# thegenemyers/FASTGA

Hardware: NVIDIA H100
Metric: Gbp aligned/sec (genome x genome) (higher is better)
Workload: dtype int32

## Files before the change

### fastga_b200/csrc/api.cu

```cuda
#include "stages.h"
#include "handles.h"
#include <vector>
#include <algorithm>
#include <string.h>
#include <chrono>

typedef unsigned long long u64;

static inline long long now_us()
{ return std::chrono::duration_cast<std::chrono::microseconds>(std::chrono::steady_clock::now().time_since_epoch()).count(); }

static fgb_timings g_timings;

struct stage_timer
{ cudaEvent_t a, b; cudaStream_t st; float *dst;
  stage_timer(float *d, cudaStream_t s) : st(s), dst(d)
    { cudaEventCreate(&a); cudaEventCreate(&b); cudaEventRecord(a,st); }
  ~stage_timer()
    { cudaEventRecord(b,st); cudaEventSynchronize(b);
      float ms = 0; cudaEventElapsedTime(&ms,a,b); *dst += ms;
      cudaEventDestroy(a); cudaEventDestroy(b);
    }
};

void fgb_timing_add(int which, float ms)
{ if (which == 0) g_timings.triples_ms += ms;
  else if (which == 1) { g_timings.extend_ms += ms; g_timings.extend_launches += 1; }
  else if (which == 3) { g_timings.merge_ms += ms; g_timings.merge_launches += 1; }
  else g_timings.d2h_ms += ms;
}

void fgb_count_launch(int n) { g_timings.launches += n; }


#include <map>
#include <unordered_map>
#include <mutex>

static std::multimap<size_t,void *> g_free;
static std::unordered_map<void *,size_t> g_live;
static std::mutex g_mem_lock;

static size_t size_class(size_t b)
{ if (b < 4096) return 4096;
  size_t p = 4096;
  while (p < b) p <<= 1;
  size_t step = p >> 4;
  return ((b + step - 1) / step) * step;
}

cudaError_t fgb_dmalloc(void **p, size_t bytes, cudaStream_t st)
{ (void) st;
  size_t c = size_class(bytes);
  std::lock_guard<std::mutex> g(g_mem_lock);
  auto it = g_free.lower_bound(c);
  if (it != g_free.end() && it->first <= c + (c >> 2))
    { *p = it->second;
      g_live[*p] = it->first;
      g_free.erase(it);
      return cudaSuccess;
    }
  cudaError_t e = cudaMalloc(p,c);
  if (e != cudaSuccess)
    { cudaGetLastError();
      for (auto &kv : g_free) cudaFree(kv.second);
      g_free.clear();
      e = cudaMalloc(p,c);
      if (e != cudaSuccess) return e;
    }
  g_live[*p] = c;
  return cudaSuccess;
}

void fgb_dfree(void *p, cudaStream_t st)
{ (void) st;
  if (p == NULL) return;
  std::lock_guard<std::mutex> g(g_mem_lock);
  auto it = g_live.find(p);
  if (it == g_live.end()) { cudaFree(p); return; }
  g_free.insert(std::make_pair(it->second,p));
  g_live.erase(it);
}

extern "C" void fgb_release_cache()
{ std::lock_guard<std::mutex> g(g_mem_lock);
  for (auto &kv : g_free) cudaFree(kv.second);
  g_free.clear();
}

extern "C" int fgb_device_alloc(long long bytes, void **out, void *stream)
{ CUDA_TRY(fgb_dmalloc(out,(size_t) (bytes > 0 ? bytes : 16),(cudaStream_t) stream)); return FGB_OK; }
extern "C" void fgb_device_free(void *p) { fgb_dfree(p,0); }

extern "C" long long fgb_device_live_bytes()
{ std::lock_guard<std::mutex> g(g_mem_lock);
  long long s = 0;
  for (auto &kv : g_live) s += (long long) kv.second;
  return s;
}

extern "C" void fgb_timings_reset() { memset(&g_timings,0,sizeof(g_timings)); }
extern "C" void fgb_timings_get(fgb_timings *out) { *out = g_timings; }


static const long long *g_sort_len;
static int LSORT(const void *l, const void *r)
{ int x = *((const int *) l), y = *((const int *) r);
  return (int) (g_sort_len[y] - g_sort_len[x]);
}

extern "C" int fgb_genome_create(const unsigned char *bps, long long bps_bytes, int ncontig,
                                 const long long *clen, const long long *boff, int want_revcomp,
                                 fgb_genome **out, void *stream)
{ cudaStream_t st = (cudaStream_t) stream;
  if (ncontig <= 0 || ncontig > 0x7fff) return FGB_ERR_LIMIT;
  std::unique_ptr<fgb_genome> g(new fgb_genome());
  g->ncontig = ncontig;
  g->clen.assign(clen,clen+ncontig);
  g->boff.assign(boff,boff+ncontig);
  g->woff.resize(ncontig+1);
  g->seqtot = 0; g->maxlen = 0;
  long long w = 2;
  for (int c = 0; c < ncontig; c++)
    { if (clen[c] >= 0x7fffffffll) return FGB_ERR_LIMIT;
      g->woff[c] = w;
      w += ((clen[c] + 31) >> 5) + 2;
      w = (w + 1) & ~1ll;
      g->seqtot += clen[c];
      if (clen[c] > g->maxlen) g->maxlen = clen[c];
    }
  g->woff[ncontig] = w;
  g->total_words = w;

  g->perm.resize(ncontig); g->crank.resize(ncontig);
  for (int c = 0; c < ncontig; c++) g->perm[c] = c;
  g_sort_len = clen;
  qsort(g->perm.data(),ncontig,sizeof(int),LSORT);
  for (int c = 0; c < ncontig; c++) g->crank[g->perm[c]] = c;

  dblock<unsigned char> d_bps;
  dblock<long long> d_boff;
  CUDA_TRY(d_bps.alloc(bps_bytes + 16,st));
  CUDA_TRY(d_boff.alloc(ncontig,st));
  CUDA_TRY(g->d_clen.alloc(ncontig,st));
  CUDA_TRY(g->d_woff.alloc(ncontig+1,st));
  CUDA_TRY(g->d_crank.alloc(ncontig,st));
  CUDA_TRY(g->d_perm.alloc(ncontig,st));
  CUDA_TRY(g->d_seq.alloc(w + 1024,st));
  if (want_revcomp) CUDA_TRY(g->d_rseq.alloc(w + 1024,st));
  { stage_timer t(&g_timings.h2d_ms,st);
    CUDA_TRY(cudaMemcpyAsync(d_bps,bps,bps_bytes,cudaMemcpyHostToDevice,st));
    CUDA_TRY(cudaMemcpyAsync(d_boff,boff,sizeof(long long)*ncontig,cudaMemcpyHostToDevice,st));
    CUDA_TRY(cudaMemcpyAsync(g->d_clen,clen,sizeof(long long)*ncontig,cudaMemcpyHostToDevice,st));
    CUDA_TRY(cudaMemcpyAsync(g->d_woff,g->woff.data(),sizeof(long long)*(ncontig+1),cudaMemcpyHostToDevice,st));
    CUDA_TRY(cudaMemcpyAsync(g->d_crank,g->crank.data(),sizeof(int)*ncontig,cudaMemcpyHostToDevice,st));
    CUDA_TRY(cudaMemcpyAsync(g->d_perm,g->perm.data(),sizeof(int)*ncontig,cudaMemcpyHostToDevice,st));
  }
  g->h2d_bytes = bps_bytes + (long long) ncontig*(3*8+2*4) + 8;
  int rc;
  { stage_timer t(&g_timings.stage_ms,st);
    rc = fgb_stage_genome_device(d_bps,d_boff,g->d_clen,g->d_woff,ncontig,w,g->d_seq,g->d_rseq,st);
  }
  CUDA_TRY(cudaStreamSynchronize(st));
  if (rc) return rc;
  *out = g.release();
  return FGB_OK;
}

extern "C" void fgb_genome_free(fgb_genome *g) { delete g; }

extern "C" int fgb_genome_perm(const fgb_genome *g, int *perm_out)
{ memcpy(perm_out,g->perm.data(),sizeof(int)*g->ncontig); return FGB_OK; }

extern "C" int fgb_genome_download(const fgb_genome *g, int rev, unsigned long long *words,
                                   long long *woff_out)
{ const u64 *src = rev ? g->d_rseq : g->d_seq;
  if (src == NULL) return FGB_ERR_ARG;
  CUDA_TRY(cudaMemcpy(words,src,sizeof(u64)*g->total_words,cudaMemcpyDeviceToHost));
  memcpy(woff_out,g->woff.data(),sizeof(long long)*(g->ncontig+1));
  return FGB_OK;
}
extern "C" long long fgb_genome_words(const fgb_genome *g) { return g->total_words; }


extern "C" void fgb_gix_free(fgb_gix *x) { delete x; }

static void gix_bytes(const fgb_genome *g, fgb_gix *x)
{ long long cum;
  x->post_bytes = 0;
  for (cum = 1; cum < g->maxlen; cum *= 256) x->post_bytes += 1;
  x->cont_bytes = 0;
  for (cum = 1; cum < 2ll*g->ncontig; cum *= 256) x->cont_bytes += 1;
}


#define GIX_FWD_ONLY 0x80000000u

struct scan_layout
{ int fsh = 0, dbits = 0;
  dblock<unsigned long long> hist;
};

static int gix_scan(const fgb_genome *g, const unsigned char *mask, unsigned plo, unsigned phi_flags,
                    dblock<rec128> &d_recs, long long *n_out, long long *nrev, unsigned long long *buck1024,
                    scan_layout &lay, cudaStream_t st)
{ int T = fgb_sc_tile();
  std::vector<int> tc, ts;
  long long npos = 0;
  for (int c = 0; c < g->ncontig; c++)
    if (g->clen[c] >= 12 && g->boff[c] >= 0 && (mask == NULL || mask[c]))
      { npos += g->clen[c] - 11;
        for (long long t0 = 0; t0 + 12 <= g->clen[c]; t0 += T)
          { tc.push_back(c); ts.push_back((int) t0); }
      }
  int ntiles = (int) tc.size();
  dblock<int> d_tc, d_ts; dblock<unsigned> d_cnt;
  dblock<u64> d_buck, d_total; dblock<unsigned char> d_tmp;
  int rc;
  u64 total = 0, rdropped = 0;
  const unsigned phi = phi_flags & ~GIX_FWD_ONLY;
  fgb_kmer_first_digit(2*npos,plo,phi > plo ? phi : plo + 1,&lay.fsh,&lay.dbits);
  const long long ncnt = (long long) ntiles << lay.dbits;
  const long long tmpb = fgb_dev_scan_tmp_bytes(ncnt);
  CUDA_TRY(lay.hist.alloc(256,st));
  CUDA_TRY(d_tc.alloc(ntiles+1,st));
  CUDA_TRY(d_ts.alloc(ntiles+1,st));
  CUDA_TRY(d_cnt.alloc(ncnt+1,st));
  CUDA_TRY(d_buck.alloc(1025,st));
  CUDA_TRY(d_total.alloc(1,st));
  CUDA_TRY(d_tmp.alloc(tmpb,st));
  CUDA_TRY(cudaMemcpyAsync(d_tc,tc.data(),sizeof(int)*ntiles,cudaMemcpyHostToDevice,st));
  CUDA_TRY(cudaMemcpyAsync(d_ts,ts.data(),sizeof(int)*ntiles,cudaMemcpyHostToDevice,st));
  { stage_timer t(&g_timings.scan_ms,st);
    rc = fgb_syncmer_digit_count_device(g->d_seq,g->d_clen,g->d_woff,g->d_crank,d_tc,d_ts,ntiles,d_buck,d_cnt,
                                        lay.fsh,lay.dbits,lay.hist,d_total,d_tmp,tmpb,plo,phi_flags,st);
    if (rc) return rc;
    CUDA_TRY(cudaMemcpyAsync(&total,d_total,8,cudaMemcpyDeviceToHost,st));
    if (buck1024) CUDA_TRY(cudaMemcpyAsync(buck1024,d_buck,8*1024,cudaMemcpyDeviceToHost,st));
    CUDA_TRY(cudaMemcpyAsync(&rdropped,d_buck + 1024,8,cudaMemcpyDeviceToHost,st));
    CUDA_TRY(cudaStreamSynchronize(st));
  }
  if (total >= 0xfffffff0ull) return FGB_ERR_LIMIT;
  dblock<rec128> d_a;
  CUDA_TRY(d_a.alloc(total+1,st));
  { stage_timer t(&g_timings.scan_ms,st);
    rc = fgb_syncmer_digit_emit_device(g->d_seq,g->d_clen,g->d_woff,g->d_crank,d_tc,d_ts,ntiles,d_cnt,lay.fsh,
                                       lay.dbits,(long long) total,d_a,plo,phi_flags,st);
  }
  if (rc) return rc;
  CUDA_TRY(cudaStreamSynchronize(st));
  d_recs = std::move(d_a); *n_out = (long long) total; *nrev = (long long) rdropped;
  return FGB_OK;
}

static int gix_finish(fgb_gix *x, dblock<rec128> d_a, long long n, unsigned plo, unsigned phi, const scan_layout &lay,
                      cudaStream_t st, bool index = true)
{ dblock<rec128> d_b; dblock<unsigned char> d_stmp;
  long long stmpb = fgb_sort128_tmp_bytes(n);
  int rc, inb = 0;
  x->n = n;
  CUDA_TRY(d_b.alloc(n+1,st));
  CUDA_TRY(d_stmp.alloc(stmpb,st));
  if (index)
    { CUDA_TRY(x->d_pstart.alloc((1<<24)+1+8,st));
      CUDA_TRY(x->d_adj.alloc((size_t) n + 32,st));
    }
  { stage_timer t(&g_timings.ksort_ms,st);
    rc = fgb_kmer_sort_device(d_a,d_b,n,plo,phi,lay.fsh,lay.dbits,lay.hist,d_stmp,stmpb,&inb,st);
  }
  if (rc) return rc;
  x->d_tab = std::move(inb ? d_b : d_a);
  if (index)
    { stage_timer t(&g_timings.index_ms,st);
      rc = fgb_kix_index_device(x->d_tab,n,x->d_pstart,x->d_adj,st);
    }
  if (rc) return rc;
  CUDA_TRY(cudaStreamSynchronize(st));
  return FGB_OK;
}

static int gix_build_range(const fgb_genome *g, unsigned plo, unsigned phi_flags, bool index, fgb_gix **out,
                           void *stream)
{ cudaStream_t st = (cudaStream_t) stream;
  const unsigned phi = phi_flags & ~GIX_FWD_ONLY;
  std::unique_ptr<fgb_gix> x(new fgb_gix());
  gix_bytes(g,x.get());
  x->ncontig = g->ncontig;
  x->fwd_only = (phi_flags & GIX_FWD_ONLY) ? 1 : 0;
  dblock<rec128> d_a; long long n = 0, nrev = 0;
  scan_layout lay;
  int rc = gix_scan(g,NULL,plo,phi_flags,d_a,&n,&nrev,x->buck1024,lay,st);
  if (rc) return rc;
  x->n_both = n + nrev;
  const char *part_env = getenv("FGB_KSORT_PARTITION");
  const bool ignore_layout = part_env != NULL && atoi(part_env) != 0;
  const scan_layout none;
  if ((rc = gix_finish(x.get(),std::move(d_a),n,plo,phi,ignore_layout ? none : lay,st,index))) return rc;
  *out = x.release();
  return FGB_OK;
}

extern "C" int fgb_gix_build(const fgb_genome *g, fgb_gix **out, void *stream)
{ return gix_build_range(g,0u,1u << 24,true,out,stream); }

extern "C" int fgb_gix_build_forward(const fgb_genome *g, fgb_gix **out, void *stream)
{ return gix_build_range(g,0u,(1u << 24) | GIX_FWD_ONLY,true,out,stream); }

extern "C" int fgb_gix_build_range(const fgb_genome *g, unsigned plo, unsigned phi, fgb_gix **out, void *stream)
{ if (plo > phi || phi > (1u << 24)) return FGB_ERR_ARG;
  return gix_build_range(g,plo,phi,true,out,stream);
}


extern "C" int fgb_kmers_scan(const fgb_genome *g, const unsigned char *mask, int fwd_only,
                              void **d_recs, long long *n, void *stream)
{ dblock<rec128> d; long long nrev = 0;
  scan_layout lay;
  int rc = gix_scan(g,mask,0u,(1u << 24) | (fwd_only ? GIX_FWD_ONLY : 0u),d,n,&nrev,NULL,lay,(cudaStream_t) stream);
  if (rc) return rc;
  *d_recs = d.release();
  return FGB_OK;
}

extern "C" int fgb_gix_from_records(const void *d_recs, long long n, unsigned plo, unsigned phi, int fwd_only,
                                    int post_bytes, int cont_bytes, int ncontig, fgb_gix **out, void *stream)
{ cudaStream_t st = (cudaStream_t) stream;
  if (n < 0 || n >= 0xfffffff0ll || plo >= phi || phi > (1u << 24)) return FGB_ERR_ARG;
  std::unique_ptr<fgb_gix> x(new fgb_gix());
  x->n_both = n; x->post_bytes = post_bytes; x->cont_bytes = cont_bytes; x->ncontig = ncontig;
  x->fwd_only = fwd_only ? 1 : 0;
  dblock<rec128> d_a;
  CUDA_TRY(d_a.alloc(n+1,st));
  if (n > 0) CUDA_TRY(cudaMemcpyAsync(d_a,d_recs,sizeof(rec128)*n,cudaMemcpyDeviceToDevice,st));
  int rc = gix_finish(x.get(),std::move(d_a),n,plo,phi,scan_layout(),st);
  if (rc) return rc;
  *out = x.release();
  return FGB_OK;
}

extern "C" long long fgb_gix_size(const fgb_gix *x) { return x->n; }
extern "C" int fgb_gix_post_bytes(const fgb_gix *x) { return x->post_bytes; }
extern "C" int fgb_gix_cont_bytes(const fgb_gix *x) { return x->cont_bytes; }

extern "C" int fgb_gix_download(const fgb_gix *x, void *tab , unsigned *pstart ,
                                unsigned long long *buck1024)
{ if (tab) CUDA_TRY(cudaMemcpy(tab,x->d_tab,sizeof(rec128)*x->n,cudaMemcpyDeviceToHost));
  if (pstart) CUDA_TRY(cudaMemcpy(pstart,x->d_pstart,sizeof(unsigned)*((1<<24)+1),cudaMemcpyDeviceToHost));
  if (buck1024) memcpy(buck1024,x->buck1024,8*1024);
  return FGB_OK;
}

extern "C" int fgb_gix_upload(const void *tab, long long n, int post_bytes, int cont_bytes,
                              int ncontig, fgb_gix **out, void *stream)
{ cudaStream_t st = (cudaStream_t) stream;
  if (n >= 0xfffffff0ll) return FGB_ERR_LIMIT;
  std::unique_ptr<fgb_gix> x(new fgb_gix());
  x->n = n; x->n_both = n; x->post_bytes = post_bytes; x->cont_bytes = cont_bytes; x->ncontig = ncontig;
  CUDA_TRY(x->d_tab.alloc(n+1,st));
  CUDA_TRY(x->d_pstart.alloc((1<<24)+1+8,st));
  CUDA_TRY(x->d_adj.alloc((size_t) x->n + 32,st));
  CUDA_TRY(cudaMemcpyAsync(x->d_tab,tab,sizeof(rec128)*n,cudaMemcpyHostToDevice,st));
  int rc = fgb_kix_index_device(x->d_tab,n,x->d_pstart,x->d_adj,st);
  CUDA_TRY(cudaStreamSynchronize(st));
  if (rc) return rc;
  *out = x.release();
  return FGB_OK;
}

extern "C" int fgb_gix_import_ktab(const unsigned char *entries, long long n, int post_bytes,
                                   int cont_bytes, const long long *index, int ncontig,
                                   fgb_gix **out, void *stream)
{ cudaStream_t st = (cudaStream_t) stream;
  if (n >= 0xfffffff0ll || post_bytes > 4 || cont_bytes > 2) return FGB_ERR_LIMIT;
  std::unique_ptr<fgb_gix> x(new fgb_gix());
  x->n = n; x->n_both = n; x->post_bytes = post_bytes; x->cont_bytes = cont_bytes; x->ncontig = ncontig;
  long long E = 9 + post_bytes + cont_bytes;
  dblock<unsigned char> d_ent; dblock<long long> d_index;
  CUDA_TRY(d_ent.alloc(E*n + 16,st));
  CUDA_TRY(d_index.alloc(1ll << 24,st));
  CUDA_TRY(x->d_tab.alloc(n+1,st));
  CUDA_TRY(x->d_pstart.alloc((1<<24)+1+8,st));
  CUDA_TRY(x->d_adj.alloc((size_t) x->n + 32,st));
  CUDA_TRY(cudaMemcpyAsync(d_ent,entries,E*n,cudaMemcpyHostToDevice,st));
  CUDA_TRY(cudaMemcpyAsync(d_index,index,8ll<<24,cudaMemcpyHostToDevice,st));
  int rc = fgb_ktab_import_device(d_ent,n,post_bytes,cont_bytes,d_index,x->d_tab,st);
  if (!rc) rc = fgb_kix_index_device(x->d_tab,n,x->d_pstart,x->d_adj,st);
  CUDA_TRY(cudaStreamSynchronize(st));
  if (rc) return rc;
  *out = x.release();
  return FGB_OK;
}

extern "C" int fgb_gix_export_ktab(const fgb_gix *x, const long long *part_first, int nparts,
                                   unsigned char *out, void *stream)
{ cudaStream_t st = (cudaStream_t) stream;
  long long E = 9 + x->post_bytes + x->cont_bytes;
  dblock<unsigned char> d_out; dblock<long long> d_pf;
  CUDA_TRY(d_out.alloc(E*x->n + 16,st));
  CUDA_TRY(d_pf.alloc(nparts+1,st));
  CUDA_TRY(cudaMemcpyAsync(d_pf,part_first,8*nparts,cudaMemcpyHostToDevice,st));
  int rc = fgb_ktab_export_device(x->d_tab,x->n,x->post_bytes,x->cont_bytes,d_pf,nparts,d_out,st);
  if (!rc) CUDA_TRY(cudaMemcpyAsync(out,d_out,E*x->n,cudaMemcpyDeviceToHost,st));
  CUDA_TRY(cudaStreamSynchronize(st));
  return rc;
}


static int bitlen(long long v) { int b = 0; while (v > 0) { b += 1; v >>= 1; } return b; }

extern "C" void fgb_seeds_free(fgb_seeds *s) { delete s; }

static int seeds_find_impl(const fgb_gix *x1, const fgb_gix *x2, long long amxpos,
                           long long bmxpos, int freq, bool self, fgb_seeds **out, void *stream);

extern "C" int fgb_seeds_find(const fgb_gix *x1, const fgb_gix *x2, long long amxpos,
                              long long bmxpos, int freq, fgb_seeds **out, void *stream)
{ return seeds_find_impl(x1,x2,amxpos,bmxpos,freq,false,out,stream); }

extern "C" int fgb_seeds_find_self(const fgb_gix *x, long long amxpos, int freq, fgb_seeds **out, void *stream)
{ return seeds_find_impl(x,x,amxpos,amxpos,freq,true,out,stream); }

struct seed_bits { int anti, band, jc, ic, key; };

static int seed_layout_of(const fgb_gix *x1, const fgb_gix *x2, long long amxpos, long long bmxpos, seed_bits *L)
{ L->anti = bitlen(amxpos + bmxpos);
  L->band = L->anti > 6 ? L->anti - 6 : 1;
  L->jc   = bitlen(x2->ncontig > 1 ? x2->ncontig-1 : 1);
  L->ic   = bitlen(x1->ncontig > 1 ? x1->ncontig-1 : 1);
  L->key  = 12 + L->anti + L->band + L->jc + L->ic + 1;
  return L->key > 128 ? FGB_ERR_LIMIT : FGB_OK;
}

static int seeds_merge_impl(const fgb_gix *x1, const fgb_gix *x2, long long amxpos, long long bmxpos, int freq,
                            bool self, const seed_bits &L, dblock<rec128> &d_out, long long *nseeds_out,
                            long long *sumlen_out, long long *n1m_out, cudaStream_t st)
{ if (self && x1->fwd_only) return FGB_ERR_ARG;
  dblock<u64> d_counters; dblock<rec128> d_fwd, d_a;
  int rc;
  u64 nseeds = 0, sumlen = 0;
  const rec128 *t1 = x1->d_tab; long long n1 = x1->n;
  CUDA_TRY(d_counters.alloc(2,st));
  if (!self && !x1->fwd_only && n1 > 0)
    { CUDA_TRY(d_fwd.alloc(n1+1,st));
      if ((rc = fgb_forward_view_device(x1->d_tab,n1,d_fwd,&n1,st))) return rc;
      t1 = d_fwd;
    }
  long long cap = (self ? 2*x1->n : 2*n1 + (n1 >> 1)) + 1024;
  for (int attempt = 0; ; attempt++)
    { CUDA_TRY(d_a.alloc(cap+1,st));
      if (self)
        rc = fgb_self_merge_device(x1->d_tab,x1->n,x1->d_pstart,freq,L.anti,L.band,L.jc,L.ic,amxpos,
                                   d_a,cap,d_counters,&nseeds,&sumlen,st);
      else
        rc = fgb_merge_device(t1,n1,x2->d_tab,x2->n,x2->d_pstart,x2->d_adj,freq,L.anti,L.band,L.jc,L.ic,
                              amxpos,bmxpos,d_a,cap,d_counters,&nseeds,&sumlen,st);
      if (rc == FGB_OK) break;
      d_a.reset();
      if (rc != FGB_ERR_OVERFLOW || attempt > 0) return rc;
      cap = (long long) nseeds + 1024;
      g_timings.merge_ms = 0; g_timings.merge_launches = 0;
    }
  if (nseeds >= 0xfffffff0ull) return FGB_ERR_LIMIT;
  d_out = std::move(d_a); *nseeds_out = (long long) nseeds; *sumlen_out = (long long) sumlen; *n1m_out = n1;
  return FGB_OK;
}

#define SEED_SORT_LO_ANY    6
#define SEED_SORT_LO_MERGED 7

static int seeds_sort_impl(dblock<rec128> d_a, long long n, const seed_bits &L, int bit_lo, long long amxpos,
                           long long bmxpos, bool self, long long sumlen, long long n1m, fgb_seeds **out,
                           cudaStream_t st)
{ dblock<rec128> d_b; dblock<unsigned char> d_tmp;
  std::unique_ptr<fgb_seeds> s(new fgb_seeds());
  s->self_mode = self ? 1 : 0;
  s->anti_bits = L.anti; s->band_bits = L.band; s->jc_bits = L.jc; s->ic_bits = L.ic;
  s->amxpos = amxpos; s->bmxpos = bmxpos;
  s->n = n; s->sumlen = sumlen; s->n1_merged = n1m;
  long long tmpb = fgb_sort128_tmp_bytes(n);
  int rc, inb = 0;
  const char *wide_env = getenv("FGB_SEED_SORT_WIDE");
  const bool narrow = L.key <= 64 && !(wide_env != NULL && atoi(wide_env) != 0);
  u64 hiflag = 0, *d_hiflag = NULL;
  CUDA_TRY(d_b.alloc(n+1,st));
  CUDA_TRY(d_tmp.alloc(tmpb,st));
  { stage_timer t(&g_timings.ssort_ms,st);
    rc = fgb_radix_sort_device(d_a,d_b,n,bit_lo,L.key,narrow,d_tmp,tmpb,&inb,&d_hiflag,st);
  }
  if (rc) return rc;
  if (d_hiflag) CUDA_TRY(cudaMemcpyAsync(&hiflag,d_hiflag,8,cudaMemcpyDeviceToHost,st));
  CUDA_TRY(cudaStreamSynchronize(st));
  if (hiflag) return FGB_ERR_ARG;
  s->d_rec = std::move(inb ? d_b : d_a);
  *out = s.release();
  return FGB_OK;
}

static int seeds_find_impl(const fgb_gix *x1, const fgb_gix *x2, long long amxpos,
                           long long bmxpos, int freq, bool self, fgb_seeds **out, void *stream)
{ cudaStream_t st = (cudaStream_t) stream;
  seed_bits L;
  int rc = seed_layout_of(x1,x2,amxpos,bmxpos,&L);
  if (rc) return rc;
  dblock<rec128> d_a; long long n = 0, sumlen = 0, n1m = 0;
  if ((rc = seeds_merge_impl(x1,x2,amxpos,bmxpos,freq,self,L,d_a,&n,&sumlen,&n1m,st))) return rc;
  return seeds_sort_impl(std::move(d_a),n,L,SEED_SORT_LO_MERGED,amxpos,bmxpos,self,sumlen,n1m,out,st);
}


extern "C" int fgb_seeds_merge(const fgb_gix *x1, const fgb_gix *x2, long long amxpos, long long bmxpos, int freq,
                               void **d_seeds, long long *n, int *bits, long long *info, void *stream)
{ seed_bits L;
  int rc = seed_layout_of(x1,x2,amxpos,bmxpos,&L);
  if (rc) return rc;
  dblock<rec128> d_a; long long sumlen = 0, n1m = 0;
  if ((rc = seeds_merge_impl(x1,x2,amxpos,bmxpos,freq,false,L,d_a,n,&sumlen,&n1m,(cudaStream_t) stream))) return rc;
  *d_seeds = d_a.release();
  bits[0] = L.anti; bits[1] = L.band; bits[2] = L.jc; bits[3] = L.ic;
  if (info) { info[0] = sumlen; info[1] = n1m; }
  return FGB_OK;
}

static int group_by_owner(const void *d_src, long long n, int pos, int nbits, const int *owner, int nowner,
                          int world, void *d_out, long long *bounds, cudaStream_t st)
{ if (world < 1 || world > 64) return FGB_ERR_ARG;
  for (int w = 0; w <= world; w++) bounds[w] = 0;
  if (n <= 0) return FGB_OK;
  dblock<int> d_owner; dblock<u64> d_cnt;
  int rc;
  u64 cnt[64], base[65];
  CUDA_TRY(d_owner.alloc((size_t) nowner,st));
  CUDA_TRY(d_cnt.alloc(64*2,st));
  CUDA_TRY(cudaMemcpyAsync(d_owner,owner,sizeof(int)*(size_t) nowner,cudaMemcpyHostToDevice,st));
  CUDA_TRY(cudaMemsetAsync(d_cnt,0,8*64*2,st));
  if ((rc = fgb_owner_count_device(d_src,n,pos,nbits,d_owner,nowner,world,d_cnt,st))) return rc;
  CUDA_TRY(cudaMemcpyAsync(cnt,d_cnt,8*64,cudaMemcpyDeviceToHost,st));
  CUDA_TRY(cudaStreamSynchronize(st));
  base[0] = 0;
  for (int w = 0; w < world; w++) base[w+1] = base[w] + cnt[w];
  CUDA_TRY(cudaMemcpyAsync(d_cnt + 64,base,8*64,cudaMemcpyHostToDevice,st));
  if ((rc = fgb_owner_scatter_device(d_src,n,pos,nbits,d_owner,nowner,world,d_cnt + 64,d_out,st))) return rc;
  CUDA_TRY(cudaStreamSynchronize(st));
  for (int w = 0; w <= world; w++) bounds[w] = (long long) base[w];
  return FGB_OK;
}

extern "C" int fgb_seeds_group_by_owner(const void *d_seeds, long long n, const int *bits, const int *owner,
                                        int nrank_contigs, int world, void *d_out, long long *bounds,
                                        void *stream)
{ return group_by_owner(d_seeds,n,12 + bits[0] + bits[1] + bits[2],bits[3],owner,nrank_contigs,world,d_out,bounds,
                        (cudaStream_t) stream);
}

extern "C" int fgb_records_group_by_owner(const void *d_recs, long long n, const int *owner256, int world,
                                          void *d_out, long long *bounds, void *stream)
{ return group_by_owner(d_recs,n,120,8,owner256,256,world,d_out,bounds,(cudaStream_t) stream); }

extern "C" int fgb_seeds_from_records(const void *d_recs, long long n, const int *bits, long long amxpos,
                                      long long bmxpos, long long sumlen, fgb_seeds **out, void *stream)
{ cudaStream_t st = (cudaStream_t) stream;
  if (n < 0 || n >= 0xfffffff0ll) return FGB_ERR_LIMIT;
  seed_bits L;
  L.anti = bits[0]; L.band = bits[1]; L.jc = bits[2]; L.ic = bits[3];
  L.key = 12 + L.anti + L.band + L.jc + L.ic + 1;
  if (L.key > 128) return FGB_ERR_LIMIT;
  dblock<rec128> d_a;
  CUDA_TRY(d_a.alloc(n+1,st));
  if (n > 0) CUDA_TRY(cudaMemcpyAsync(d_a,d_recs,sizeof(rec128)*n,cudaMemcpyDeviceToDevice,st));
  return seeds_sort_impl(std::move(d_a),n,L,SEED_SORT_LO_ANY,amxpos,bmxpos,false,sumlen,0,out,st);
}

extern "C" long long fgb_seeds_size(const fgb_seeds *s) { return s->n; }
extern "C" long long fgb_seeds_sumlen(const fgb_seeds *s) { return s->sumlen; }
extern "C" int fgb_seeds_layout(const fgb_seeds *s, int *bits )
{ bits[0] = s->anti_bits; bits[1] = s->band_bits; bits[2] = s->jc_bits; bits[3] = s->ic_bits; return FGB_OK; }
extern "C" int fgb_seeds_download(const fgb_seeds *s, void *rec)
{ CUDA_TRY(cudaMemcpy(rec,s->d_rec,sizeof(rec128)*s->n,cudaMemcpyDeviceToHost)); return FGB_OK; }

extern "C" int fgb_sort128_host(void *recs, long long n, int byte_lo, int byte_hi, void *stream)
{ cudaStream_t st = (cudaStream_t) stream;
  dblock<rec128> d_a, d_b; dblock<unsigned char> d_tmp;
  long long tmpb = fgb_sort128_tmp_bytes(n);
  CUDA_TRY(d_a.alloc(n+1,st));
  CUDA_TRY(d_b.alloc(n+1,st));
  CUDA_TRY(d_tmp.alloc(tmpb,st));
  CUDA_TRY(cudaMemcpyAsync(d_a,recs,sizeof(rec128)*n,cudaMemcpyHostToDevice,st));
  int inb = 0;
  int rc = fgb_sort128_device(d_a,d_b,n,byte_lo,byte_hi,d_tmp,tmpb,&inb,st);
  if (!rc) CUDA_TRY(cudaMemcpyAsync(recs,inb ? d_b : d_a,sizeof(rec128)*n,cudaMemcpyDeviceToHost,st));
  CUDA_TRY(cudaStreamSynchronize(st));
  return rc;
}

extern "C" int fgb_device_ready()
{ int n = 0;
  if (cudaGetDeviceCount(&n) != cudaSuccess || n == 0) return 0;
  return 1;
}


struct fgb_run_stats
{ long long nkmers1, nkmers2, nseeds, sumlen, nhits, nla, nwaves, ncells, nraw, h2d_bytes, d2h_bytes,
            nseg, nwork, warp_cycles, wave_cycles, extract_cycles,
            us_gix, us_seeds, us_extend, us_filter, nkmers1_fwd,
            slow_cycles, slow_waves, paired_waves, pairings; };

static int align_pipeline(const fgb_genome *A, const fgb_genome *B, bool self, const float *freqA, int freq,
                          int chain_break, int chain_min, int align_min, double align_rate, fgb_alns **out,
                          fgb_run_stats *stats, cudaStream_t st)
{ fgb_run_stats s = {};
  fgb_seeds *ps = NULL; fgb_overlaps *po = NULL;
  int rc;
  long long t0 = now_us(), t1, t2, t3, t4;
  { std::unique_ptr<fgb_gix> x1, x2;
    fgb_gix *p = NULL;
    if ((rc = gix_build_range(A,0u,(1u << 24) | (self ? 0u : GIX_FWD_ONLY),self,&p,st))) return rc;
    x1.reset(p);
    if (!self)
      { if ((rc = gix_build_range(B,0u,1u << 24,true,&p,st))) return rc;
        x2.reset(p);
      }
    const fgb_gix *xb = self ? x1.get() : x2.get();
    t1 = now_us();
    s.nkmers1 = x1->n_both; s.nkmers2 = xb->n;
    seed_bits L;
    dblock<rec128> d_a; long long n = 0;
    rc = seed_layout_of(x1.get(),xb,A->maxlen,B->maxlen,&L);
    if (!rc) rc = seeds_merge_impl(x1.get(),xb,A->maxlen,B->maxlen,freq,self,L,d_a,&n,&s.sumlen,&s.nkmers1_fwd,st);
    x1.reset(); x2.reset();
    if (!rc) rc = seeds_sort_impl(std::move(d_a),n,L,SEED_SORT_LO_MERGED,A->maxlen,B->maxlen,self,s.sumlen,
                                  s.nkmers1_fwd,&ps,st);
  }
  if (rc) return rc;
  std::unique_ptr<fgb_seeds> sd(ps);
  s.nseeds = sd->n;
  t2 = now_us();
  std::vector<short> tables(65536);
  int ave = 0;
  fgb_align_spec(1.-align_rate,freqA,tables.data(),&ave);
  rc = fgb_extend(sd.get(),A,B,chain_break,chain_min,align_min,align_rate,tables.data(),ave,100,&po,st);
  t3 = now_us();
  const int jb = sd->jc_bits, ib = sd->ic_bits;
  sd.reset();
  if (rc) return rc;
  std::unique_ptr<fgb_overlaps> ov(po);
  rc = fgb_filter(ov.get(),A->perm.data(),B->perm.data(),jb,ib,1,out);
  t4 = now_us();
  unsigned long long c[16];
  fgb_overlaps_counters(ov.get(),c);
  s.us_gix = t1-t0; s.us_seeds = t2-t1; s.us_extend = t3-t2; s.us_filter = t4-t3;
  s.nhits = (long long) c[0]; s.nla = (long long) c[1]; s.nwaves = (long long) c[2]; s.ncells = (long long) c[3];
  s.nseg = (long long) c[5]; s.nwork = (long long) c[6];
  s.warp_cycles = (long long) c[8]; s.wave_cycles = (long long) c[9]; s.extract_cycles = (long long) c[10];
  s.slow_cycles = (long long) ((c[15] >> 40) << 12); s.slow_waves = (long long) ((c[15] >> 16) & 0xffffff);
  s.paired_waves = (long long) c[11]; s.pairings = (long long) c[12];
  s.h2d_bytes = A->h2d_bytes + (self ? 0 : B->h2d_bytes) + 65536*2;
  s.d2h_bytes = fgb_overlaps_bytes(ov.get()) + 16 + 8*1024*(self ? 1 : 2) + 64;
  if (stats) *stats = s;
  return rc;
}

extern "C" int fgb_align_resident(const fgb_genome *A, const fgb_genome *B, const float *freqA,
                                  int freq, int chain_break, int chain_min, int align_min,
                                  double align_rate, fgb_alns **out, fgb_run_stats *stats, void *stream)
{ return align_pipeline(A,B,false,freqA,freq,chain_break,chain_min,align_min,align_rate,out,stats,
                        (cudaStream_t) stream);
}

extern "C" int fgb_fastga_self(const unsigned char *bps, long long nb, int nc, const long long *clen,
                               const long long *boff, const float *freq4,
                               int freq, int chain_break, int chain_min, int align_min, double align_rate,
                               fgb_alns **out, fgb_run_stats *stats, void *stream)
{ fgb_genome *p = NULL;
  int rc;
  if ((rc = fgb_genome_create(bps,nb,nc,clen,boff,1,&p,stream))) return rc;
  std::unique_ptr<fgb_genome> A(p);
  return align_pipeline(A.get(),A.get(),true,freq4,freq,chain_break,chain_min,align_min,align_rate,out,stats,
                        (cudaStream_t) stream);
}

extern "C" int fgb_fastga(const unsigned char *bpsA, long long nbA, int ncA, const long long *clenA,
                          const long long *boffA, const float *freqA,
                          const unsigned char *bpsB, long long nbB, int ncB, const long long *clenB,
                          const long long *boffB,
                          int freq, int chain_break, int chain_min, int align_min, double align_rate,
                          fgb_alns **out, fgb_run_stats *stats, void *stream)
{ fgb_genome *p = NULL;
  int rc;
  if ((rc = fgb_genome_create(bpsA,nbA,ncA,clenA,boffA,1,&p,stream))) return rc;
  std::unique_ptr<fgb_genome> A(p);
  if ((rc = fgb_genome_create(bpsB,nbB,ncB,clenB,boffB,0,&p,stream))) return rc;
  std::unique_ptr<fgb_genome> B(p);
  return align_pipeline(A.get(),B.get(),false,freqA,freq,chain_break,chain_min,align_min,align_rate,out,stats,
                        (cudaStream_t) stream);
}
```

### fastga_b200/csrc/common.cuh

```cuda
#pragma once
#include <cuda_runtime.h>
#include <stdint.h>
#include <stdio.h>
#include <stdlib.h>

#define FGB_OK            0
#define FGB_ERR_CUDA     -1
#define FGB_ERR_ARG      -2
#define FGB_ERR_LIMIT    -3
#define FGB_ERR_OVERFLOW -4

#define CUDA_TRY(call)                                                                   \
  do { cudaError_t _e = (call);                                                          \
       if (_e != cudaSuccess)                                                            \
         { fprintf(stderr,"fastga_b200: CUDA error %s at %s:%d: %s\n",                   \
                   cudaGetErrorName(_e),__FILE__,__LINE__,cudaGetErrorString(_e));       \
           return FGB_ERR_CUDA; } } while (0)

struct __align__(16) rec128 { unsigned long long lo, hi; };

static __device__ __forceinline__ rec128 ld_rec(const rec128 *p)
{ uint4 v = *reinterpret_cast<const uint4 *>(p);
  rec128 r;
  r.lo = (unsigned long long) v.x | ((unsigned long long) v.y << 32);
  r.hi = (unsigned long long) v.z | ((unsigned long long) v.w << 32);
  return r;
}

static __device__ __forceinline__ void st_rec(rec128 *p, rec128 r)
{ uint4 v;
  v.x = (unsigned) r.lo; v.y = (unsigned) (r.lo >> 32);
  v.z = (unsigned) r.hi; v.w = (unsigned) (r.hi >> 32);
  *reinterpret_cast<uint4 *>(p) = v;
}

static __device__ __forceinline__ unsigned rec_byte(const rec128 &r, int b)
{ return (b < 8) ? (unsigned) ((r.lo >> (8*b)) & 0xff) : (unsigned) ((r.hi >> (8*(b-8))) & 0xff); }

static __device__ __forceinline__ unsigned rec_dig(const rec128 &r, int sh)
{ if (sh >= 64) return (unsigned) ((r.hi >> (sh - 64)) & 0xff);
  if (sh <= 56) return (unsigned) ((r.lo >> sh) & 0xff);
  return (unsigned) (((r.lo >> sh) | (r.hi << (64 - sh))) & 0xff);
}

static __device__ __forceinline__ unsigned lanemask_lt()
{ unsigned m; asm volatile("mov.u32 %0, %%lanemask_lt;" : "=r"(m)); return m; }

#define KREC_PREFIX24(hi)   ((unsigned) ((hi) >> 40))
#define KREC_SUFFIX56(r)    ((((r).hi & 0xffffffffffull) << 16) | ((r).lo >> 48))

int fgb_dev_exclusive_scan_u32(unsigned *d_data, long long n, unsigned long long *d_total,
                               void *d_tmp, long long tmp_bytes, cudaStream_t st);
long long fgb_dev_scan_tmp_bytes(long long n);

void fgb_timing_add(int which, float ms);
void fgb_count_launch(int n);

cudaError_t fgb_dmalloc(void **p, size_t bytes, cudaStream_t st);
void fgb_dfree(void *p, cudaStream_t st);

template<class T> struct dblock
{ dblock() = default;
  dblock(const dblock &) = delete;
  dblock &operator=(const dblock &) = delete;
  dblock(dblock &&o) noexcept : p(o.p), st(o.st) { o.p = nullptr; }
  dblock &operator=(dblock &&o) noexcept
    { if (this != &o) { reset(); p = o.p; st = o.st; o.p = nullptr; } return *this; }
  ~dblock() { reset(); }
  cudaError_t alloc(size_t count, cudaStream_t s)
    { reset();
      void *q = nullptr;
      cudaError_t e = fgb_dmalloc(&q,sizeof(T)*count,s);
      if (e == cudaSuccess) { p = (T *) q; st = s; }
      return e;
    }
  void reset() { if (p != nullptr) { fgb_dfree(p,st); p = nullptr; } }
  T *release() { T *q = p; p = nullptr; return q; }
  operator T *() const { return p; }
private:
  T *p = nullptr;
  cudaStream_t st = 0;
};

static __device__ __forceinline__ unsigned smem_u32(const void *p)
{ return (unsigned) __cvta_generic_to_shared(p); }

static __device__ __forceinline__ void mbar_init(unsigned long long *bar, int count)
{ asm volatile("mbarrier.init.shared::cta.b64 [%0], %1;" :: "r"(smem_u32(bar)), "r"(count) : "memory");
  asm volatile("fence.mbarrier_init.release.cluster;" ::: "memory");
  asm volatile("fence.proxy.async.shared::cta;" ::: "memory");
}

static __device__ __forceinline__ void tma_load_1d(void *smem_dst, const void *gmem_src, unsigned bytes,
                                                   unsigned long long *bar)
{ asm volatile("mbarrier.arrive.expect_tx.shared::cta.b64 _, [%0], %1;"
               :: "r"(smem_u32(bar)), "r"(bytes) : "memory");
  asm volatile("cp.async.bulk.shared::cluster.global.mbarrier::complete_tx::bytes [%0], [%1], %2, [%3];"
               :: "r"(smem_u32(smem_dst)), "l"(gmem_src), "r"(bytes), "r"(smem_u32(bar)) : "memory");
}

static __device__ __forceinline__ void mbar_expect_tx(unsigned long long *bar, unsigned bytes)
{ asm volatile("mbarrier.arrive.expect_tx.shared::cta.b64 _, [%0], %1;"
               :: "r"(smem_u32(bar)), "r"(bytes) : "memory");
}

static __device__ __forceinline__ void tma_copy_1d(void *smem_dst, const void *gmem_src, unsigned bytes,
                                                   unsigned long long *bar)
{ asm volatile("cp.async.bulk.shared::cluster.global.mbarrier::complete_tx::bytes [%0], [%1], %2, [%3];"
               :: "r"(smem_u32(smem_dst)), "l"(gmem_src), "r"(bytes), "r"(smem_u32(bar)) : "memory");
}

static __device__ __forceinline__ void mbar_wait(unsigned long long *bar, unsigned phase)
{ unsigned ok;
  do
    asm volatile("{ .reg .pred p; mbarrier.try_wait.parity.shared::cta.b64 p, [%1], %2; selp.u32 %0, 1, 0, p; }"
                 : "=r"(ok) : "r"(smem_u32(bar)), "r"(phase) : "memory");
  while (!ok);
}
```

### fastga_b200/csrc/sort128.cu

```cuda
#include "stages.h"
#include <stdlib.h>
#include <utility>
#include <vector>

#define SORT_THREADS 512
#ifndef SORT_ITEMS
#define SORT_ITEMS   8
#endif
#ifndef SORT64_ITEMS
#define SORT64_ITEMS 16
#endif
#ifndef SORT_MINBLK
#define SORT_MINBLK  2
#endif
#define SORT_TILE    (SORT_THREADS*SORT_ITEMS)
#define SORT_WARPS   (SORT_THREADS/32)
static_assert(SORT_THREADS*SORT64_ITEMS >= SORT_TILE, "fgb_sort128_tmp_bytes sizes the look-back status for SORT_TILE");

typedef unsigned long long u64;

static __device__ __forceinline__ unsigned warp_incl_scan(unsigned v, int lane)
{
#pragma unroll
  for (int o = 1; o < 32; o <<= 1)
    { unsigned t = __shfl_up_sync(0xffffffffu,v,o);
      if (lane >= o) v += t;
    }
  return v;
}

static __device__ __forceinline__ unsigned rec_dig(u64 v, int sh) { return (unsigned) (v >> sh) & 0xff; }
static __device__ __forceinline__ u64 ld_rec(const u64 *p) { return *p; }
static __device__ __forceinline__ void st_rec(u64 *p, u64 v) { *p = v; }



static __device__ __forceinline__ unsigned match_digit(unsigned d, bool valid)
{ unsigned peers = __ballot_sync(0xffffffffu,valid);
#pragma unroll
  for (int k = 0; k < 8; k++)
    { bool bit = (d >> k) & 1;
      unsigned bk = __ballot_sync(0xffffffffu,bit);
      peers &= bit ? bk : ~bk;
    }
  return peers;
}

static __device__ __forceinline__ unsigned warp_rank(unsigned *myc, unsigned d, bool valid)
{ const int lane = threadIdx.x & 31;
  unsigned peers = match_digit(d,valid);
  int leader = valid ? __ffs(peers)-1 : lane;
  unsigned b = 0;
  if (valid && lane == leader)
    { b = myc[d];
      myc[d] = b + __popc(peers);
    }
  b = __shfl_sync(0xffffffffu,b,leader);
  __syncwarp();
  return b + __popc(peers & lanemask_lt());
}

template <class F>
static __device__ __forceinline__ unsigned digit_offsets(unsigned *wcount, unsigned *bexcl, unsigned *wtot, F publish)
{ const int tid = threadIdx.x, lane = tid & 31, w = tid >> 5;
  unsigned c = 0, inc = 0;
  __syncthreads();
  if (tid < 256)
    {
#pragma unroll
      for (int ww = 0; ww < SORT_WARPS; ww++)
        { unsigned t = wcount[ww*256+tid];
          wcount[ww*256+tid] = c;
          c += t;
        }
      publish(c);
      inc = warp_incl_scan(c,lane);
      if (lane == 31) wtot[w] = inc;
    }
  __syncthreads();
  if (tid < 256)
    { unsigned pre = 0;
      for (int i = 0; i < w; i++) pre += wtot[i];
      bexcl[tid] = pre + inc - c;
    }
  __syncthreads();
  return c;
}

#define ST_AGG  (1ull << 62)
#define ST_INC  (2ull << 62)
#define ST_MASK ((1ull << 62) - 1)

static __device__ __forceinline__ u64 lookback(const u64 *status, unsigned tileid, int tid)
{ volatile const u64 *stt = status;
  u64 excl = 0;
  for (long long t = (long long) tileid - 1; t >= 0; )
    { u64 v[4];
#pragma unroll
      for (int q = 0; q < 4; q++)
        v[q] = (t - q >= 0) ? stt[(u64) (t - q)*256 + tid] : ST_INC;
      bool done = false;
#pragma unroll
      for (int q = 0; q < 4; q++)
        { if (done || (v[q] >> 62) == 0) break;
          excl += v[q] & ST_MASK;
          t -= 1;
          if (v[q] & ST_INC) done = true;
        }
      if (done) break;
    }
  return excl;
}

__global__ void __launch_bounds__(SORT_THREADS)
sort_ghist_kernel(const rec128 *__restrict__ in, long long n, int dsh , unsigned long long *__restrict__ ghist)
{ __shared__ unsigned h[256];
  int tid = threadIdx.x;
  if (tid < 256) h[tid] = 0;
  __syncthreads();
  const bool one = (dsh >= 64 || dsh <= 56);
  const unsigned long long *half = reinterpret_cast<const unsigned long long *>(in) + (dsh >= 64);
  const int sh = dsh & 63;
  for (long long tile0 = (long long) blockIdx.x * SORT_TILE; tile0 < n; tile0 += (long long) gridDim.x * SORT_TILE)
    {
#pragma unroll
      for (int it = 0; it < SORT_ITEMS; it++)
        { long long idx = tile0 + it*SORT_THREADS + tid;
          bool valid = idx < n;
          unsigned d = 0;
          if (valid) d = one ? (unsigned) ((half[2*idx] >> sh) & 0xff) : rec_dig(ld_rec(in + idx),dsh);
          unsigned peers = match_digit(d,valid);
          if (valid && (tid & 31) == __ffs(peers)-1) atomicAdd(&h[d],__popc(peers));
        }
    }
  __syncthreads();
  if (tid < 256 && h[tid]) atomicAdd(&ghist[tid],(unsigned long long) h[tid]);
}

__global__ void sort_bins_kernel(const unsigned long long *__restrict__ ghist, unsigned long long *__restrict__ binbase,
                                 unsigned long long *__restrict__ nexthist, unsigned *__restrict__ ticket)
{ __shared__ unsigned long long ws[8];
  int tid = threadIdx.x, lane = tid & 31, w = tid >> 5;
  unsigned long long v = ghist[tid], inc = v;
  for (int o = 1; o < 32; o <<= 1)
    { unsigned long long t = __shfl_up_sync(0xffffffffu,inc,o);
      if (lane >= o) inc += t;
    }
  if (lane == 31) ws[w] = inc;
  __syncthreads();
  unsigned long long pre = 0;
  for (int i = 0; i < w; i++) pre += ws[i];
  binbase[tid] = pre + inc - v;
  nexthist[tid] = 0;
  if (tid == 0) *ticket = 0;
}

template <int IW> struct os_tile
{ static constexpr int ITEMS = (IW == 16) ? SORT_ITEMS : SORT64_ITEMS;
  static constexpr int TILE  = SORT_THREADS*ITEMS;
  static constexpr size_t SMEM = (size_t) TILE*IW + (SORT_WARPS*256 + 256 + 256 + 8)*sizeof(unsigned)
                                 + 256*sizeof(u64);
};

template <class Key, int IW, int OW>
__global__ void __launch_bounds__(SORT_THREADS,SORT_MINBLK)
sort_onesweep_kernel(const void *__restrict__ in, void *__restrict__ out, long long n, int dsh ,
                     int next_dsh , const u64 *__restrict__ binbase,
                     u64 *__restrict__ nexthist, u64 *status , unsigned *__restrict__ ticket,
                     u64 *__restrict__ hiflag)
{ constexpr int ITEMS = os_tile<IW>::ITEMS, TILE = os_tile<IW>::TILE;
  extern __shared__ __align__(16) unsigned char smem_raw[];
  Key      *tile   = reinterpret_cast<Key *>(smem_raw);
  unsigned *wcount = reinterpret_cast<unsigned *>(smem_raw + (size_t) TILE*IW);
  unsigned *bexcl  = wcount + SORT_WARPS*256;
  unsigned *nhist  = bexcl + 256;
  unsigned *wtot   = nhist + 256;
  u64      *gbase  = reinterpret_cast<u64 *>(wtot + 8);
  __shared__ unsigned tile_s;
  __shared__ __align__(8) u64 tbar;

  int tid = threadIdx.x, lane = tid & 31, w = tid >> 5;
  if (tid == 0)
    { unsigned t = atomicAdd(ticket,1u);
      tile_s = t;
      long long t0 = (long long) t * TILE, rm = n - t0;
      unsigned nb = ((unsigned) (rm < TILE ? rm : TILE) * IW + 15u) & ~15u;
      mbar_init(&tbar,1);
      tma_load_1d(tile,reinterpret_cast<const unsigned char *>(in) + t0*IW,nb,&tbar);
    }
  for (int i = tid; i < SORT_WARPS*256; i += SORT_THREADS) wcount[i] = 0;
  if (tid < 256) nhist[tid] = 0;
  __syncthreads();
  const unsigned tileid = tile_s;
  long long tile0 = (long long) tileid * TILE;
  long long rem = n - tile0;
  int cnt = rem < TILE ? (int) rem : TILE;

  Key      r[ITEMS];
  unsigned rank[ITEMS];
  u64      hi_or = 0;
  int base = w*(32*ITEMS);
  unsigned *myc = wcount + w*256;
  mbar_wait(&tbar,0);
#pragma unroll
  for (int it = 0; it < ITEMS; it++)
    { int idx = base + it*32 + lane;
      bool valid = idx < cnt;
      unsigned d = 0;
      if (valid)
        { if constexpr (sizeof(Key) < IW)
            { rec128 v = ld_rec(reinterpret_cast<const rec128 *>(smem_raw) + idx);
              r[it] = v.lo;
              hi_or |= v.hi;
            }
          else
            r[it] = ld_rec(tile + idx);
          d = rec_dig(r[it],dsh);
        }
      rank[it] = warp_rank(myc,d,valid);
      if (next_dsh >= 0 && valid) atomicAdd(&nhist[rec_dig(r[it],next_dsh)],1u);
    }
  if (sizeof(Key) < IW && hi_or) atomicOr(hiflag,hi_or);

  u64 *mine = status + (u64) tileid*256 + tid;
  const unsigned c = digit_offsets(wcount,bexcl,wtot,[&](unsigned total)
    { if (tileid == 0)
        atomicExch(mine,ST_INC | total);
      else
        atomicExch(mine,ST_AGG | total);
    });

#pragma unroll
  for (int it = 0; it < ITEMS; it++)
    { int idx = base + it*32 + lane;
      if (idx < cnt)
        { unsigned d = rec_dig(r[it],dsh);
          st_rec(tile + (bexcl[d] + myc[d] + rank[it]),r[it]);
        }
    }
  if (tid < 256)
    { u64 excl = lookback(status,tileid,tid);
      if (tileid != 0) atomicExch(mine,ST_INC | (excl + c));
      gbase[tid] = binbase[tid] + excl - bexcl[tid];
      if (next_dsh >= 0 && nhist[tid]) atomicAdd(&nexthist[tid],(u64) nhist[tid]);
    }
  __syncthreads();

  for (int p = tid; p < cnt; p += SORT_THREADS)
    { Key v = ld_rec(tile + p);
      u64 o = gbase[rec_dig(v,dsh)] + p;
      if constexpr (sizeof(Key) < OW)
        { rec128 R; R.lo = v; R.hi = 0;
          st_rec(reinterpret_cast<rec128 *>(out) + o,R);
        }
      else
        st_rec(reinterpret_cast<Key *>(out) + o,v);
    }
}

struct sort_tmp
{ u64 *status, *hist[2], *binbase, *hiflag;
  unsigned *ticket;
  sort_tmp(void *d_tmp, long long n)
    { long long ntiles = (n + SORT_TILE - 1) / SORT_TILE;
      if (ntiles < 1) ntiles = 1;
      status  = (u64 *) d_tmp;
      hist[0] = status + 256ull*ntiles;
      hist[1] = hist[0] + 256;
      binbase = hist[1] + 256;
      ticket  = (unsigned *) (binbase + 256);
      hiflag  = binbase + 256 + 1;
    }
};

extern "C" long long fgb_sort128_tmp_bytes(long long n)
{ long long ntiles = (n + SORT_TILE - 1) / SORT_TILE;
  if (ntiles < 1) ntiles = 1;
  return 256*ntiles*8 + (3*256 + 16)*8;
}

static int first_pass_hist(const void *d_a, long long n, int dsh, const sort_tmp &T, cudaStream_t st)
{ CUDA_TRY(cudaMemsetAsync(T.hist[0],0,256*8,st));
  int ntiles = (int) ((n + SORT_TILE - 1) / SORT_TILE), nb = ntiles < 1184 ? ntiles : 1184;
  sort_ghist_kernel<<<nb,SORT_THREADS,0,st>>>((const rec128 *) d_a,n,dsh,T.hist[0]);
  fgb_count_launch(1);
  return FGB_OK;
}

template <class Key, int IW, int OW>
static int onesweep_pass(const void *in, void *out, long long n, int dsh, int next_dsh, const sort_tmp &T, int cur,
                         cudaStream_t st)
{ typedef os_tile<IW> O;
  static bool attr_set = false;
  if (!attr_set)
    { CUDA_TRY(cudaFuncSetAttribute(sort_onesweep_kernel<Key,IW,OW>,cudaFuncAttributeMaxDynamicSharedMemorySize,(int) O::SMEM));
      attr_set = true;
    }
  int ntiles = (int) ((n + O::TILE - 1) / O::TILE);
  sort_bins_kernel<<<1,256,0,st>>>(T.hist[cur],T.binbase,T.hist[cur^1],T.ticket);
  CUDA_TRY(cudaMemsetAsync(T.status,0,256ull*ntiles*8,st));
  sort_onesweep_kernel<Key,IW,OW><<<ntiles,SORT_THREADS,O::SMEM,st>>>(in,out,n,dsh,next_dsh,T.binbase,T.hist[cur^1],
                                                                     T.status,T.ticket,T.hiflag);
  fgb_count_launch(2);
  return FGB_OK;
}

extern "C" int fgb_radix_sort_device(void *d_a, void *d_b, long long n, int bit_lo, int bit_hi, int narrow,
                                     void *d_tmp, long long tmp_bytes, int *result_in_b, u64 **d_hiflag, void *stream)
{ cudaStream_t st = (cudaStream_t) stream;
  if (n < 0 || bit_lo < 0 || bit_hi > (narrow ? 64 : 128) || bit_lo > bit_hi) return FGB_ERR_ARG;
  if (n >= 0xffffffffll) return FGB_ERR_LIMIT;
  *result_in_b = 0;
  const sort_tmp T(d_tmp,n);
  if (narrow)
    { if (tmp_bytes < fgb_sort128_tmp_bytes(n)) return FGB_ERR_ARG;
      CUDA_TRY(cudaMemsetAsync(T.hiflag,0,8,st));
      *d_hiflag = T.hiflag;
    }
  if (n <= 1 || bit_lo == bit_hi) return FGB_OK;
  if (tmp_bytes < fgb_sort128_tmp_bytes(n)) return FGB_ERR_ARG;

  const int npass = (bit_hi - bit_lo + 7) / 8;
  const bool words = narrow && npass >= 2;
  void *half[2] = { d_b, (unsigned char *) d_b + ((8*n + 15) & ~15ll) };

  int rc = first_pass_hist(d_a,n,bit_lo,T,st);
  for (int p = 0; p < npass && rc == FGB_OK; p++)
    { const int b = bit_lo + 8*p, nd = (p + 1 < npass) ? b + 8 : -1, cur = p & 1;
      if (!words)
        rc = onesweep_pass<rec128,16,16>(cur ? d_b : d_a,cur ? d_a : d_b,n,b,nd,T,cur,st);
      else if (p == 0)
        rc = onesweep_pass<u64,16,8>(d_a,half[0],n,b,nd,T,cur,st);
      else if (nd >= 0)
        rc = onesweep_pass<u64,8,8>(half[cur^1],half[cur],n,b,nd,T,cur,st);
      else
        rc = onesweep_pass<u64,8,16>(half[cur^1],d_a,n,b,nd,T,cur,st);
    }
  if (rc) return rc;
  CUDA_TRY(cudaGetLastError());
  if (!words && (npass & 1))
    { if (narrow)
        CUDA_TRY(cudaMemcpyAsync(d_a,d_b,sizeof(rec128)*n,cudaMemcpyDeviceToDevice,st));
      else
        *result_in_b = 1;
    }
  return FGB_OK;
}

extern "C" int fgb_sort128_device(void *d_a, void *d_b, long long n, int byte_lo, int byte_hi,
                                  void *d_tmp, long long tmp_bytes, int *result_in_b, void *stream)
{ if (byte_lo < 0 || byte_hi > 16 || byte_lo > byte_hi) return FGB_ERR_ARG;
  return fgb_radix_sort_device(d_a,d_b,n,8*byte_lo,8*byte_hi,0,d_tmp,tmp_bytes,result_in_b,NULL,stream);
}


#define BK_THREADS SORT_THREADS
#define BK_ITEMS   8
#define BK_CAP     (BK_THREADS*BK_ITEMS)
#define BK_WARPS   SORT_WARPS
#define BK_SPAN    4
#define BK_SUBBITS 10
#define BK_NSUB    (BK_SPAN << BK_SUBBITS)
#define BK_MAXSUB  32

__global__ void kmer_bins_kernel(const rec128 *__restrict__ tab, long long n, int binshift, unsigned long long base,
                                 unsigned *__restrict__ bin_start, long long nbins)
{ long long i = (long long) blockIdx.x * blockDim.x + threadIdx.x;
  if (i > n) return;
  long long lo = (i == 0) ? -1 : (long long) ((tab[i-1].hi >> binshift) - base);
  long long hi = (i == n) ? nbins : (long long) ((tab[i].hi >> binshift) - base);
  if (hi > nbins) hi = nbins;
  for (long long p = lo+1; p <= hi; p++) bin_start[p] = (unsigned) i;
}


__global__ void __launch_bounds__(BK_THREADS,2)
kmer_bucket_sort_kernel(const rec128 *__restrict__ in, rec128 *__restrict__ out,
                        const uint4 *__restrict__ groups ,
                        int binshift)
{ extern __shared__ __align__(16) unsigned char smem_raw[];
  rec128   *tile   = reinterpret_cast<rec128 *>(smem_raw);
  unsigned *cnt    = reinterpret_cast<unsigned *>(tile + BK_CAP);
  unsigned *bexcl  = cnt + BK_NSUB + 32;
  unsigned *wtot   = bexcl + 256;
  __shared__ __align__(8) unsigned long long tbar;

  const int tid = threadIdx.x, lane = tid & 31, w = tid >> 5;
  const uint4 g = groups[blockIdx.x];
  const int count = (int) g.y;
  if (tid == 0)
    { mbar_init(&tbar,1);
      tma_load_1d(tile,in + g.x,(unsigned) count * 16u,&tbar);
    }
  for (int i = tid; i <= BK_NSUB; i += BK_THREADS) cnt[i] = 0;
  __syncthreads();
  mbar_wait(&tbar,0);

  rec128   r[BK_ITEMS];
  unsigned sub[BK_ITEMS], off[BK_ITEMS];
  const int base = w*(32*BK_ITEMS);
  const unsigned b0 = g.z;
  const int subshift = binshift - BK_SUBBITS;
#pragma unroll
  for (int it = 0; it < BK_ITEMS; it++)
    { int idx = base + it*32 + lane;
      if (idx < count)
        { r[it] = ld_rec(tile + idx);
          sub[it] = ((((unsigned) (r[it].hi >> binshift)) - b0) << BK_SUBBITS) | ((unsigned) (r[it].hi >> subshift) & ((1u << BK_SUBBITS)-1));
          off[it] = atomicAdd(&cnt[sub[it]],1u);
        }
    }
  __syncthreads();
  bool big = false;
  { unsigned v[8], sum = 0;
#pragma unroll
    for (int i = 0; i < 8; i++) { v[i] = cnt[8*tid+i]; big |= (v[i] > BK_MAXSUB); sum += v[i]; }
    unsigned inc = warp_incl_scan(sum,lane);
    if (lane == 31) wtot[w] = inc;
    __syncthreads();
    unsigned pre = inc - sum;
    for (int i = 0; i < w; i++) pre += wtot[i];
#pragma unroll
    for (int i = 0; i < 8; i++) { cnt[8*tid+i] = pre; pre += v[i]; }
    if (tid == BK_THREADS-1) cnt[BK_NSUB] = pre;
  }
  big = __syncthreads_or(big);

  if (!big)
    {
#pragma unroll
      for (int it = 0; it < BK_ITEMS; it++)
        { int idx = base + it*32 + lane;
          if (idx < count) st_rec(tile + (cnt[sub[it]] + off[it]),r[it]);
        }
      __syncthreads();
      for (int p = tid; p < count; p += BK_THREADS)
        { rec128 R = ld_rec(tile + p);
          unsigned sb = ((((unsigned) (R.hi >> binshift)) - b0) << BK_SUBBITS) | ((unsigned) (R.hi >> subshift) & ((1u << BK_SUBBITS)-1));
          int s = (int) cnt[sb], e = (int) cnt[sb+1], rank = 0;
          for (int q = s; q < e; q++)
            { rec128 Q = ld_rec(tile + q);
              bool less = (Q.hi < R.hi) || (Q.hi == R.hi && (Q.lo < R.lo || (Q.lo == R.lo && q < p)));
              rank += less;
            }
          st_rec(out + (g.x + s + rank),R);
        }
      return;
    }

  unsigned *wcount = cnt;
  unsigned *myc = wcount + w*256;
  unsigned rank[BK_ITEMS];
  __syncthreads();
#pragma unroll
  for (int i = 0; i < 8; i++) myc[i*32 + lane] = 0;
  __syncwarp();
  for (int byte = 0; byte < 16; byte++)
    {
#pragma unroll
      for (int it = 0; it < BK_ITEMS; it++)
        { int idx = base + it*32 + lane;
          bool valid = idx < count;
          rank[it] = warp_rank(myc,valid ? rec_byte(r[it],byte) : 0,valid);
        }
      digit_offsets(wcount,bexcl,wtot,[](unsigned) {});
#pragma unroll
      for (int it = 0; it < BK_ITEMS; it++)
        { int idx = base + it*32 + lane;
          if (idx < count)
            { unsigned d = rec_byte(r[it],byte);
              st_rec(tile + (bexcl[d] + myc[d] + rank[it]),r[it]);
            }
        }
      __syncthreads();
      if (byte + 1 < 16)
        {
#pragma unroll
          for (int it = 0; it < BK_ITEMS; it++)
            { int idx = base + it*32 + lane;
              if (idx < count) r[it] = ld_rec(tile + idx);
            }
#pragma unroll
          for (int i = 0; i < 8; i++) myc[i*32 + lane] = 0;
          __syncwarp();
        }
    }
  for (int p = tid; p < count; p += BK_THREADS)
    st_rec(out + (g.x + p),ld_rec(tile + p));
}

__global__ void kmer_copy_segments_kernel(const rec128 *__restrict__ src, rec128 *__restrict__ dst,
                                          const unsigned *__restrict__ sfrom, const unsigned *__restrict__ dfrom,
                                          const unsigned *__restrict__ pre, int nseg, long long total)
{ for (long long i = (long long) blockIdx.x * blockDim.x + threadIdx.x; i < total;
       i += (long long) gridDim.x * blockDim.x)
    { int lo = 0, hi = nseg;
      while (hi - lo > 1) { int md = (lo+hi) >> 1; if (pre[md] <= i) lo = md; else hi = md; }
      unsigned o = (unsigned) (i - pre[lo]);
      st_rec(dst + (dfrom[lo] + o),ld_rec(src + (sfrom[lo] + o)));
    }
}

static const size_t BUCKET_SMEM = BK_CAP*sizeof(rec128) + (BK_NSUB + 32 + 256 + BK_WARPS)*sizeof(unsigned);

extern "C" int fgb_kmer_bin_shift(long long n, unsigned plo, unsigned phi)
{ long long maxbins = 65536, target = 1536;
  if (getenv("FGB_KSORT_BIN_TARGET") != NULL) target = atoll(getenv("FGB_KSORT_BIN_TARGET"));
  if (target < 1) target = 1;
  while (maxbins < (1ll << 24) && n / maxbins > target) maxbins <<= 1;
  int sh = 0;
  while ((long long) ((((unsigned long long) (phi - 1) >> sh) - ((unsigned long long) plo >> sh))) >= maxbins) sh += 1;
  return sh;
}

extern "C" void fgb_kmer_first_digit(long long nmax, unsigned plo, unsigned phi, int *fsh, int *dbits)
{ *fsh = fgb_kmer_bin_shift(nmax,plo,phi);
  int bits = 24 - *fsh, passes = (bits - 9 + 7) / 8;
  if (passes < 1) passes = 1;
  *dbits = bits - 8*passes;
}

static int kmer_sort_binned(const rec128 *src, rec128 *dst, const unsigned *bins, long long nbins, int sh,
                            unsigned plo, cudaStream_t st)
{ const int binshift = 40 + sh;
  const unsigned base = plo >> sh;
  int rc = FGB_OK;
  static bool attr_set = false;
  if (!attr_set)
    { CUDA_TRY(cudaFuncSetAttribute(kmer_bucket_sort_kernel,cudaFuncAttributeMaxDynamicSharedMemorySize,
                                    (int) BUCKET_SMEM));
      attr_set = true;
    }

  std::vector<uint4> groups;
  std::vector<unsigned> ofrom, opre;
  unsigned ototal = 0;
  { unsigned gs = bins[0], gc = 0; long long gp = 0;
    for (long long p = 0; p < nbins; p++)
      { unsigned len = bins[p+1] - bins[p];
        if (len == 0) continue;
        if (len > BK_CAP)
          { if (gc) { groups.push_back(make_uint4(gs,gc,base + (unsigned) gp,0)); gc = 0; }
            ofrom.push_back(bins[p]); opre.push_back(ototal); ototal += len;
            continue;
          }
        if (gc != 0 && (gc + len > BK_CAP || p - gp >= BK_SPAN))
          { groups.push_back(make_uint4(gs,gc,base + (unsigned) gp,0)); gc = 0; }
        if (gc == 0) { gs = bins[p]; gp = p; }
        gc += len;
      }
    if (gc) groups.push_back(make_uint4(gs,gc,base + (unsigned) gp,0));
  }

  dblock<uint4> d_groups;
  if (!groups.empty())
    { CUDA_TRY(d_groups.alloc(groups.size(),st));
      CUDA_TRY(cudaMemcpyAsync(d_groups,groups.data(),sizeof(uint4)*groups.size(),cudaMemcpyHostToDevice,st));
      kmer_bucket_sort_kernel<<<(unsigned) groups.size(),BK_THREADS,BUCKET_SMEM,st>>>(src,dst,d_groups,binshift);
      fgb_count_launch(1);
      CUDA_TRY(cudaGetLastError());
    }
  if (ototal > 0)
    { int nseg = (int) ofrom.size();
      opre.push_back(ototal);
      std::vector<unsigned> cfrom(opre.begin(),opre.end()-1);
      dblock<rec128> d_c1, d_c2; dblock<unsigned char> d_ctmp; dblock<unsigned> d_seg;
      long long ctb = fgb_sort128_tmp_bytes(ototal);
      CUDA_TRY(d_c1.alloc((size_t) ototal+1,st));
      CUDA_TRY(d_c2.alloc((size_t) ototal+1,st));
      CUDA_TRY(d_ctmp.alloc(ctb,st));
      CUDA_TRY(d_seg.alloc(3*(size_t) nseg+1,st));
      CUDA_TRY(cudaMemcpyAsync(d_seg,ofrom.data(),sizeof(unsigned)*nseg,cudaMemcpyHostToDevice,st));
      CUDA_TRY(cudaMemcpyAsync(d_seg+nseg,cfrom.data(),sizeof(unsigned)*nseg,cudaMemcpyHostToDevice,st));
      CUDA_TRY(cudaMemcpyAsync(d_seg+2*nseg,opre.data(),sizeof(unsigned)*(nseg+1),cudaMemcpyHostToDevice,st));
      int nb = (int) ((ototal + 255) / 256); if (nb > 4736) nb = 4736;
      kmer_copy_segments_kernel<<<nb,256,0,st>>>(src,d_c1,d_seg,d_seg+nseg,d_seg+2*nseg,nseg,ototal);
      int cinb = 0;
      rc = fgb_sort128_device(d_c1,d_c2,ototal,0,16,d_ctmp,ctb,&cinb,st);
      if (rc) return rc;
      kmer_copy_segments_kernel<<<nb,256,0,st>>>(cinb ? d_c2 : d_c1,dst,d_seg+nseg,d_seg,d_seg+2*nseg,nseg,ototal);
      fgb_count_launch(2);
      CUDA_TRY(cudaGetLastError());
      CUDA_TRY(cudaStreamSynchronize(st));
    }
  CUDA_TRY(cudaStreamSynchronize(st));
  return FGB_OK;
}

extern "C" int fgb_kmer_sort_device(void *d_a, void *d_b, long long n, unsigned plo, unsigned phi, int fsh, int dbits,
                                    const u64 *d_hist, void *d_tmp, long long tmp_bytes, int *result_in_b, void *stream)
{ cudaStream_t st = (cudaStream_t) stream;
  *result_in_b = 0;
  if (n <= 1) return FGB_OK;
  if (n >= 0xffffffffll) return FGB_ERR_LIMIT;
  if (phi <= plo || phi > (1u << 24) || tmp_bytes < fgb_sort128_tmp_bytes(n)) return FGB_ERR_ARG;
  const int sh = fgb_kmer_bin_shift(n,plo,phi);
  if (dbits == 0) fsh = sh;
  if (sh < fsh) return FGB_ERR_ARG;
  const sort_tmp T(d_tmp,n);
  const int b0 = 64 + 40 + fsh + dbits, npass = (128 - b0 + 7) / 8;
  if (dbits == 0)
    { int rc = first_pass_hist(d_a,n,b0,T,st);
      if (rc) return rc;
    }
  else
    CUDA_TRY(cudaMemcpyAsync(T.hist[0],d_hist,256*8,cudaMemcpyDeviceToDevice,st));
  rec128 *src = (rec128 *) d_a, *dst = (rec128 *) d_b;
  for (int p = 0; p < npass; p++)
    { const int b = b0 + 8*p, nd = (p + 1 < npass) ? b + 8 : -1;
      int rc = onesweep_pass<rec128,16,16>(src,dst,n,b,nd,T,p & 1,st);
      if (rc) return rc;
      std::swap(src,dst);
    }
  CUDA_TRY(cudaGetLastError());

  const unsigned long long base = (unsigned long long) plo >> sh, fbase = (unsigned long long) plo >> fsh;
  const long long nf = (long long) (((unsigned long long) (phi - 1) >> fsh) - fbase) + 1;
  const long long nbins = (long long) (((unsigned long long) (phi - 1) >> sh) - base) + 1;
  std::vector<unsigned> fstart((size_t) nf + 1), bins((size_t) nbins + 1);
  { dblock<unsigned> d_fstart;
    CUDA_TRY(d_fstart.alloc((size_t) (nf+1),st));
    kmer_bins_kernel<<<(int) ((n + 1 + 255) / 256),256,0,st>>>(src,n,40 + fsh,fbase,d_fstart,nf);
    fgb_count_launch(1);
    CUDA_TRY(cudaMemcpyAsync(fstart.data(),d_fstart,sizeof(unsigned)*(size_t) (nf+1),cudaMemcpyDeviceToHost,st));
    CUDA_TRY(cudaStreamSynchronize(st));
  }
  for (long long p = 0; p <= nbins; p++)
    { long long f = (long long) ((base + p) << (sh - fsh)) - (long long) fbase;
      bins[p] = fstart[f < 0 ? 0 : (f > nf ? nf : f)];
    }
  int rc = kmer_sort_binned(src,dst,bins.data(),nbins,sh,plo,st);
  if (rc) return rc;
  *result_in_b = (dst == (rec128 *) d_b);
  return FGB_OK;
}


#define SCAN_THREADS 1024
#define SCAN_ITEMS   8
#define SCAN_TILE    (SCAN_THREADS*SCAN_ITEMS)

__global__ void __launch_bounds__(SCAN_THREADS)
scan_reduce_kernel(const unsigned *__restrict__ data, long long n, unsigned long long *__restrict__ sums)
{ __shared__ unsigned long long ws[32];
  long long t0 = (long long) blockIdx.x * SCAN_TILE;
  unsigned long long s = 0;
  for (int i = 0; i < SCAN_ITEMS; i++)
    { long long idx = t0 + i*SCAN_THREADS + threadIdx.x;
      if (idx < n) s += data[idx];
    }
  for (int o = 16; o > 0; o >>= 1) s += __shfl_down_sync(0xffffffffu,s,o);
  if ((threadIdx.x & 31) == 0) ws[threadIdx.x >> 5] = s;
  __syncthreads();
  if (threadIdx.x < 32)
    { s = ws[threadIdx.x];
      for (int o = 16; o > 0; o >>= 1) s += __shfl_down_sync(0xffffffffu,s,o);
      if (threadIdx.x == 0) sums[blockIdx.x] = s;
    }
}

__global__ void __launch_bounds__(1024)
scan_sums_kernel(unsigned long long *__restrict__ sums, int nb, unsigned long long *__restrict__ total)
{ __shared__ unsigned long long ws[32];
  __shared__ unsigned long long carry_s;
  int tid = threadIdx.x, lane = tid & 31, w = tid >> 5;
  if (tid == 0) carry_s = 0;
  __syncthreads();
  for (int base = 0; base < nb; base += 1024)
    { int i = base + tid;
      unsigned long long v = (i < nb) ? sums[i] : 0, inc = v;
      for (int o = 1; o < 32; o <<= 1)
        { unsigned long long t = __shfl_up_sync(0xffffffffu,inc,o);
          if (lane >= o) inc += t;
        }
      if (lane == 31) ws[w] = inc;
      __syncthreads();
      if (w == 0)
        { unsigned long long s = ws[lane], si = s;
          for (int o = 1; o < 32; o <<= 1)
            { unsigned long long t = __shfl_up_sync(0xffffffffu,si,o);
              if (lane >= o) si += t;
            }
          ws[lane] = si - s;
        }
      __syncthreads();
      unsigned long long ex = carry_s + ws[w] + inc - v;
      if (i < nb) sums[i] = ex;
      __syncthreads();
      if (tid == 1023) carry_s = ex + v;
      __syncthreads();
    }
  if (tid == 0 && total != NULL) *total = carry_s;
}

__global__ void __launch_bounds__(SCAN_THREADS)
scan_down_kernel(unsigned *__restrict__ data, long long n, const unsigned long long *__restrict__ sums)
{ __shared__ unsigned ws[32];
  int tid = threadIdx.x, lane = tid & 31, w = tid >> 5;
  long long t0 = (long long) blockIdx.x * SCAN_TILE + (long long) tid * SCAN_ITEMS;
  unsigned v[SCAN_ITEMS], s = 0;
#pragma unroll
  for (int i = 0; i < SCAN_ITEMS; i++)
    { v[i] = (t0 + i < n) ? data[t0+i] : 0;
      s += v[i];
    }
  unsigned inc = warp_incl_scan(s,lane);
  if (lane == 31) ws[w] = inc;
  __syncthreads();
  if (w == 0)
    { unsigned x = ws[lane];
      unsigned xi = warp_incl_scan(x,lane);
      ws[lane] = xi - x;
    }
  __syncthreads();
  unsigned ex = (unsigned) sums[blockIdx.x] + ws[w] + inc - s;
#pragma unroll
  for (int i = 0; i < SCAN_ITEMS; i++)
    { if (t0 + i < n) data[t0+i] = ex;
      ex += v[i];
    }
}

long long fgb_dev_scan_tmp_bytes(long long n)
{ long long nb = (n + SCAN_TILE - 1) / SCAN_TILE;
  if (nb < 1) nb = 1;
  return nb * 8 + 64;
}


int fgb_dev_exclusive_scan_u32(unsigned *d_data, long long n, unsigned long long *d_total,
                               void *d_tmp, long long tmp_bytes, cudaStream_t st)
{ if (n <= 0)
    { if (d_total) CUDA_TRY(cudaMemsetAsync(d_total,0,8,st));
      return FGB_OK;
    }
  if (tmp_bytes < fgb_dev_scan_tmp_bytes(n)) return FGB_ERR_ARG;
  int nb = (int) ((n + SCAN_TILE - 1) / SCAN_TILE);
  unsigned long long *sums = (unsigned long long *) d_tmp;
  scan_reduce_kernel<<<nb,SCAN_THREADS,0,st>>>(d_data,n,sums);
  scan_sums_kernel<<<1,1024,0,st>>>(sums,nb,d_total);
  scan_down_kernel<<<nb,SCAN_THREADS,0,st>>>(d_data,n,sums);
  fgb_count_launch(3);
  CUDA_TRY(cudaGetLastError());
  return FGB_OK;
}
```

### fastga_b200/csrc/stages.h

```cpp
#pragma once
#include "common.cuh"

struct fgb_genome;
struct fgb_seeds;
struct fgb_overlaps;
struct fgb_alns;

extern "C" {

long long fgb_sort128_tmp_bytes(long long n);
int fgb_radix_sort_device(void *d_a, void *d_b, long long n, int bit_lo, int bit_hi, int narrow,
                          void *d_tmp, long long tmp_bytes, int *result_in_b, unsigned long long **d_hiflag,
                          void *stream);
int fgb_sort128_device(void *d_a, void *d_b, long long n, int byte_lo, int byte_hi,
                       void *d_tmp, long long tmp_bytes, int *result_in_b, void *stream);
int fgb_kmer_bin_shift(long long n, unsigned plo, unsigned phi);
void fgb_kmer_first_digit(long long nmax, unsigned plo, unsigned phi, int *fsh, int *dbits);
int fgb_kmer_sort_device(void *d_a, void *d_b, long long n, unsigned plo, unsigned phi, int fsh, int dbits,
                         const unsigned long long *d_hist, void *d_tmp, long long tmp_bytes, int *result_in_b,
                         void *stream);

int fgb_stage_genome_device(const void *d_bps, const long long *d_boff, const long long *d_clen,
                            const long long *d_woff, int ncontig, long long total_words,
                            void *d_seq, void *d_rseq, void *stream);
int fgb_syncmer_digit_count_device(const void *d_seq, const long long *d_clen, const long long *d_woff,
                                   const int *d_crank, const int *d_tile_contig, const int *d_tile_start,
                                   int ntiles, unsigned long long *d_buck1024, unsigned *d_dmat, int dsh, int dbits,
                                   unsigned long long *d_nhist, unsigned long long *d_total, void *d_tmp,
                                   long long tmp_bytes, unsigned plo, unsigned phi, void *stream);
int fgb_syncmer_digit_emit_device(const void *d_seq, const long long *d_clen, const long long *d_woff,
                                  const int *d_crank, const int *d_tile_contig, const int *d_tile_start,
                                  int ntiles, unsigned *d_dmat, int dsh, int dbits, long long n, void *d_records,
                                  unsigned plo, unsigned phi, void *stream);
int fgb_kix_index_device(const void *d_tab, long long n, unsigned *d_pstart, unsigned char *d_adj, void *stream);
int fgb_ktab_export_device(const void *d_tab, long long n, int pbytes, int cbytes,
                           const long long *d_part_first, int nparts, void *d_out, void *stream);
int fgb_ktab_import_device(const void *d_ent, long long n, int pbytes, int cbytes,
                           const long long *d_index, void *d_tab, void *stream);
int fgb_sc_tile();

int fgb_forward_view_device(const void *d_T, long long n, void *d_out, long long *h_nfwd, void *stream);
int fgb_self_merge_device(const void *d_T, long long n, const unsigned *d_pstart, int freq,
                          int anti_bits, int band_bits, int jc_bits, int ic_bits,
                          long long amxpos, void *d_seeds, long long capacity,
                          unsigned long long *d_counters, unsigned long long *h_nseeds,
                          unsigned long long *h_sumlen, void *stream);
int fgb_merge_device(const void *d_T1, long long n1, const void *d_T2, long long n2, const unsigned *d_pstart2,
                     const unsigned char *d_adj2, int freq, int anti_bits, int band_bits, int jc_bits, int ic_bits,
                     long long amxpos, long long bmxpos, void *d_seeds, long long capacity,
                     unsigned long long *d_counters, unsigned long long *h_nseeds,
                     unsigned long long *h_sumlen, void *stream);
int fgb_owner_count_device(const void *d_seeds, long long n, int p_ic, int ic_bits, const int *d_owner, int nrc,
                           int world, unsigned long long *d_cnt, void *stream);
int fgb_owner_scatter_device(const void *d_seeds, long long n, int p_ic, int ic_bits, const int *d_owner, int nrc,
                             int world, unsigned long long *d_base, void *d_out, void *stream);

int fgb_extend(const fgb_seeds *S, const fgb_genome *A, const fgb_genome *B, int chain_break,
               int chain_min, int align_min, double align_rate, const short *tables, int ave_path,
               int tspace, fgb_overlaps **out, void *stream);
int fgb_align_spec(double ave_corr, const float *freq, short *tables, int *ave_path);
long long fgb_overlaps_bytes(const fgb_overlaps *o);
const unsigned char *fgb_overlaps_data(const fgb_overlaps *o);
void fgb_overlaps_counters(const fgb_overlaps *o, unsigned long long *out);
void fgb_overlaps_retry_info(const fgb_overlaps *o, long long out[4]);
int fgb_filter(const fgb_overlaps *O, const int *perm1, const int *perm2, int jc_bits, int ic_bits,
               int do_filter, fgb_alns **out);

}
```

### fastga_b200/lib.py

```python
import ctypes as C

import numpy as np

from . import load_library

c_void_p, c_int, c_ll = C.c_void_p, C.c_int, C.c_longlong

ERRORS = {-1: "CUDA runtime error", -2: "bad argument", -3: "input exceeds a device-layout limit",
          -4: "device arena overflow"}


class FgbError(RuntimeError):
    pass


def _check(rc, what):
    if rc != 0:
        raise FgbError("%s failed: %s (%d)" % (what, ERRORS.get(rc, "?"), rc))


class Timings(C.Structure):
    _fields_ = [(n, C.c_float) for n in
                ("h2d_ms", "stage_ms", "scan_ms", "ksort_ms", "index_ms", "merge_ms", "ssort_ms",
                 "triples_ms", "extend_ms", "d2h_ms", "filter_ms")] + \
               [("merge_launches", C.c_int), ("extend_launches", C.c_int), ("launches", C.c_int)]

    def asdict(self):
        return {n: getattr(self, n) for n, _ in self._fields_}


def _ptr(a):
    return a.ctypes.data_as(c_void_p)


def timings_reset():
    load_library().fgb_timings_reset()


def timings_get():
    t = Timings()
    load_library().fgb_timings_get(C.byref(t))
    return t.asdict()


def device_ready():
    return bool(load_library().fgb_device_ready())


def device_live_bytes():
    L = load_library()
    L.fgb_device_live_bytes.restype = c_ll
    L.fgb_device_live_bytes.argtypes = []
    return L.fgb_device_live_bytes()


class DeviceGenome:

    def __init__(self, genome, want_revcomp=False, stream=None):
        L = load_library()
        self.genome = genome
        self.h = c_void_p()
        L.fgb_genome_create.argtypes = [c_void_p, c_ll, c_int, c_void_p, c_void_p, c_int,
                                        C.POINTER(c_void_p), c_void_p]
        _check(L.fgb_genome_create(_ptr(genome.bps), genome.bps.size, genome.ncontig,
                                   _ptr(genome.clen), _ptr(genome.boff), int(want_revcomp),
                                   C.byref(self.h), stream), "fgb_genome_create")
        self.perm = np.zeros(genome.ncontig, dtype=np.int32)
        L.fgb_genome_perm.argtypes = [c_void_p, c_void_p]
        L.fgb_genome_perm(self.h, _ptr(self.perm))
        self.crank = np.empty_like(self.perm)
        self.crank[self.perm] = np.arange(genome.ncontig, dtype=np.int32)

    def download(self, rev=False):
        L = load_library()
        L.fgb_genome_words.restype = c_ll
        L.fgb_genome_words.argtypes = [c_void_p]
        n = L.fgb_genome_words(self.h)
        words = np.zeros(n, dtype=np.uint64)
        woff = np.zeros(self.genome.ncontig + 1, dtype=np.int64)
        L.fgb_genome_download.argtypes = [c_void_p, c_int, c_void_p, c_void_p]
        _check(L.fgb_genome_download(self.h, int(rev), _ptr(words), _ptr(woff)), "fgb_genome_download")
        return words, woff

    def close(self):
        if self.h:
            L = load_library()
            L.fgb_genome_free.argtypes = [c_void_p]
            L.fgb_genome_free(self.h)
            self.h = c_void_p()

    def __del__(self):
        try:
            self.close()
        except Exception:
            pass


class DeviceGix:

    def __init__(self, handle):
        self.h = handle

    @classmethod
    def build(cls, dgenome, stream=None):
        L = load_library()
        h = c_void_p()
        L.fgb_gix_build.argtypes = [c_void_p, C.POINTER(c_void_p), c_void_p]
        _check(L.fgb_gix_build(dgenome.h, C.byref(h), stream), "fgb_gix_build")
        return cls(h)

    @classmethod
    def build_forward(cls, dgenome, stream=None):
        L = load_library()
        h = c_void_p()
        L.fgb_gix_build_forward.argtypes = [c_void_p, C.POINTER(c_void_p), c_void_p]
        _check(L.fgb_gix_build_forward(dgenome.h, C.byref(h), stream), "fgb_gix_build_forward")
        return cls(h)

    @classmethod
    def build_range(cls, dgenome, plo, phi, stream=None):
        L = load_library()
        h = c_void_p()
        L.fgb_gix_build_range.argtypes = [c_void_p, C.c_uint, C.c_uint, C.POINTER(c_void_p), c_void_p]
        _check(L.fgb_gix_build_range(dgenome.h, plo, phi, C.byref(h), stream), "fgb_gix_build_range")
        return cls(h)

    @classmethod
    def upload(cls, tab, post_bytes, cont_bytes, ncontig, stream=None):
        L = load_library()
        h = c_void_p()
        tab = np.ascontiguousarray(tab, dtype=np.uint64).reshape(-1, 2)
        L.fgb_gix_upload.argtypes = [c_void_p, c_ll, c_int, c_int, c_int, C.POINTER(c_void_p), c_void_p]
        _check(L.fgb_gix_upload(_ptr(tab), tab.shape[0], post_bytes, cont_bytes, ncontig,
                                C.byref(h), stream), "fgb_gix_upload")
        return cls(h)

    @classmethod
    def import_ktab(cls, gixfile, stream=None):
        L = load_library()
        h = c_void_p()
        L.fgb_gix_import_ktab.argtypes = [c_void_p, c_ll, c_int, c_int, c_void_p, c_int,
                                          C.POINTER(c_void_p), c_void_p]
        ent = np.ascontiguousarray(gixfile.entries)
        idx = np.ascontiguousarray(gixfile.index, dtype=np.int64)
        _check(L.fgb_gix_import_ktab(_ptr(ent), gixfile.n, gixfile.post_bytes, gixfile.cont_bytes,
                                     _ptr(idx), gixfile.ncontig, C.byref(h), stream),
               "fgb_gix_import_ktab")
        return cls(h)

    @property
    def n(self):
        L = load_library()
        L.fgb_gix_size.restype = c_ll
        L.fgb_gix_size.argtypes = [c_void_p]
        return L.fgb_gix_size(self.h)

    @property
    def post_bytes(self):
        L = load_library()
        L.fgb_gix_post_bytes.argtypes = [c_void_p]
        return L.fgb_gix_post_bytes(self.h)

    @property
    def cont_bytes(self):
        L = load_library()
        L.fgb_gix_cont_bytes.argtypes = [c_void_p]
        return L.fgb_gix_cont_bytes(self.h)

    def download(self, want_index=True):
        L = load_library()
        n = self.n
        tab = np.zeros((n, 2), dtype=np.uint64)
        pstart = np.zeros((1 << 24) + 1, dtype=np.uint32) if want_index else None
        buck = np.zeros(1024, dtype=np.uint64)
        L.fgb_gix_download.argtypes = [c_void_p, c_void_p, c_void_p, c_void_p]
        _check(L.fgb_gix_download(self.h, _ptr(tab), _ptr(pstart) if want_index else None, _ptr(buck)),
               "fgb_gix_download")
        return tab, pstart, buck

    def export_ktab(self, part_first, stream=None):
        L = load_library()
        E = 9 + self.post_bytes + self.cont_bytes
        out = np.zeros(self.n * E, dtype=np.uint8)
        pf = np.ascontiguousarray(part_first, dtype=np.int64)
        L.fgb_gix_export_ktab.argtypes = [c_void_p, c_void_p, c_int, c_void_p, c_void_p]
        _check(L.fgb_gix_export_ktab(self.h, _ptr(pf), len(pf), _ptr(out), stream), "fgb_gix_export_ktab")
        return out

    def close(self):
        if self.h:
            L = load_library()
            L.fgb_gix_free.argtypes = [c_void_p]
            L.fgb_gix_free(self.h)
            self.h = c_void_p()

    def __del__(self):
        try:
            self.close()
        except Exception:
            pass


class DeviceSeeds:

    def __init__(self, handle):
        self.h = handle

    @classmethod
    def find(cls, gix1, gix2, amxpos, bmxpos, freq=10, stream=None):
        L = load_library()
        h = c_void_p()
        L.fgb_seeds_find.argtypes = [c_void_p, c_void_p, c_ll, c_ll, c_int, C.POINTER(c_void_p), c_void_p]
        _check(L.fgb_seeds_find(gix1.h, gix2.h, amxpos, bmxpos, freq, C.byref(h), stream), "fgb_seeds_find")
        return cls(h)

    @classmethod
    def find_self(cls, gix, amxpos, freq=10, stream=None):
        L = load_library()
        h = c_void_p()
        L.fgb_seeds_find_self.argtypes = [c_void_p, c_ll, c_int, C.POINTER(c_void_p), c_void_p]
        _check(L.fgb_seeds_find_self(gix.h, amxpos, freq, C.byref(h), stream), "fgb_seeds_find_self")
        return cls(h)

    @property
    def n(self):
        L = load_library()
        L.fgb_seeds_size.restype = c_ll
        L.fgb_seeds_size.argtypes = [c_void_p]
        return L.fgb_seeds_size(self.h)

    @property
    def sumlen(self):
        L = load_library()
        L.fgb_seeds_sumlen.restype = c_ll
        L.fgb_seeds_sumlen.argtypes = [c_void_p]
        return L.fgb_seeds_sumlen(self.h)

    @property
    def layout(self):
        L = load_library()
        bits = (c_int * 4)()
        L.fgb_seeds_layout.argtypes = [c_void_p, c_void_p]
        L.fgb_seeds_layout(self.h, bits)
        return tuple(bits)

    def download(self):
        L = load_library()
        rec = np.zeros((self.n, 2), dtype=np.uint64)
        L.fgb_seeds_download.argtypes = [c_void_p, c_void_p]
        _check(L.fgb_seeds_download(self.h, _ptr(rec)), "fgb_seeds_download")
        return rec

    def close(self):
        if self.h:
            L = load_library()
            L.fgb_seeds_free.argtypes = [c_void_p]
            L.fgb_seeds_free(self.h)
            self.h = c_void_p()

    def __del__(self):
        try:
            self.close()
        except Exception:
            pass


def sort128_host(recs, byte_lo, byte_hi, stream=None):
    L = load_library()
    assert recs.dtype == np.uint64 and recs.flags.c_contiguous and recs.shape[1] == 2
    L.fgb_sort128_host.argtypes = [c_void_p, c_ll, c_int, c_int, c_void_p]
    _check(L.fgb_sort128_host(_ptr(recs), recs.shape[0], byte_lo, byte_hi, stream), "fgb_sort128_host")
    return recs


OVL_DT = np.dtype([("triple", "i4"), ("seq", "i4"), ("pairkey", "i4"), ("abpos", "i4"), ("bbpos", "i4"),
                   ("aepos", "i4"), ("bepos", "i4"), ("diffs", "i4"), ("tlen", "i4"), ("toff", "i8")])


def align_spec(ave_corr, freq):
    L = load_library()
    tables = np.zeros(65536, dtype=np.int16)
    ave = c_int()
    f = np.ascontiguousarray(freq, dtype=np.float32)
    L.fgb_align_spec.argtypes = [C.c_double, c_void_p, c_void_p, C.POINTER(c_int)]
    _check(L.fgb_align_spec(float(ave_corr), _ptr(f), _ptr(tables), C.byref(ave)), "fgb_align_spec")
    return tables, ave.value


class DeviceOverlaps:

    def __init__(self, handle):
        self.h = handle

    @classmethod
    def extend(cls, seeds, dgenomeA, dgenomeB, freq, chain_break=2000, chain_min=170, align_min=100,
               align_rate=0.3, tspace=100, stream=None):
        L = load_library()
        tables, ave = align_spec(1.0 - align_rate, freq)
        h = c_void_p()
        L.fgb_extend.argtypes = [c_void_p, c_void_p, c_void_p, c_int, c_int, c_int, C.c_double, c_void_p,
                                 c_int, c_int, C.POINTER(c_void_p), c_void_p]
        _check(L.fgb_extend(seeds.h, dgenomeA.h, dgenomeB.h, chain_break, chain_min, align_min,
                            float(align_rate), _ptr(tables), ave, tspace, C.byref(h), stream), "fgb_extend")
        return cls(h)

    def counters(self):
        L = load_library()
        out = (C.c_ulonglong * 16)()
        L.fgb_overlaps_counters.argtypes = [c_void_p, c_void_p]
        L.fgb_overlaps_counters(self.h, out)
        v = list(out)
        return {"hits": v[0], "la_calls": v[1], "waves": v[2], "cells": v[3], "nseg": v[5], "nwork": v[6],
                "warp_cycles": v[8], "wave_cycles": v[9], "extract_cycles": v[10], "paired_waves": v[11], "pairings": v[12],
                "front_wait": v[4], "front_total": v[7], "back_wait": v[13],
                "max_warp_cycles": v[14],
                "slowest_warp": {"cycles": (v[15] >> 40) << 12, "waves": (v[15] >> 16) & 0xffffff, "la_calls": v[15] & 0xffff}}

    def retry_info(self):
        L = load_library()
        out = (C.c_longlong * 4)()
        L.fgb_overlaps_retry_info.argtypes = [c_void_p, c_void_p]
        L.fgb_overlaps_retry_info(self.h, out)
        return {"launches": out[0], "reasons": out[1], "regrowths": out[2], "reruns": out[3]}

    def records(self):
        L = load_library()
        L.fgb_overlaps_bytes.restype = c_ll
        L.fgb_overlaps_bytes.argtypes = [c_void_p]
        L.fgb_overlaps_data.restype = c_void_p
        L.fgb_overlaps_data.argtypes = [c_void_p]
        nb = L.fgb_overlaps_bytes(self.h)
        if nb == 0:
            return np.zeros(0, dtype=OVL_DT), np.zeros(0, dtype=np.uint8)
        buf = np.ctypeslib.as_array(C.cast(L.fgb_overlaps_data(self.h), C.POINTER(C.c_uint8)), shape=(nb,)).copy()
        recs = []
        off = 0
        while off < nb:
            h = np.frombuffer(buf[off:off + 40].tobytes(), dtype=np.int32)
            recs.append((h[0], h[1], h[2], h[3], h[4], h[5], h[6], h[7], h[8], off + 40))
            off += 40 + ((int(h[8]) + 7) & ~7)
        arr = np.array(recs, dtype=OVL_DT)
        order = np.lexsort((arr["seq"], arr["triple"]))
        return arr[order], buf

    def close(self):
        if self.h:
            L = load_library()
            L.fgb_overlaps_free.argtypes = [c_void_p]
            L.fgb_overlaps_free(self.h)
            self.h = c_void_p()

    def __del__(self):
        try:
            self.close()
        except Exception:
            pass


ALN_FIELDS = ("comp", "aread", "bread", "abpos", "bbpos", "aepos", "bepos", "diffs", "tlen")


class Alignments:

    def __init__(self, fields, toff, pool, nraw):
        self.fields = fields
        self.toff = toff
        self.pool = pool
        self.nraw = nraw

    def __len__(self):
        return self.fields.shape[0]

    def trace(self, i):
        return self.pool[int(self.toff[i]):int(self.toff[i]) + int(self.fields[i, 8])]

    def canonical_lines(self):
        return sorted(self.canonical_lines_unsorted())

    def canonical_lines_unsorted(self):
        out = []
        for i in range(len(self)):
            comp, ar, br, ab, bb, ae, be, df, tl = (int(x) for x in self.fields[i])
            t = self.trace(i)
            line = "A %d %d %d %d %d %d" % (ar, ab, ae, br, bb, be)
            if comp:
                line += " | R"
            line += " | D %d" % df
            line += " | T %d" % (tl // 2) + "".join(" %d" % v for v in t[1::2])
            line += " | X %d" % (tl // 2) + "".join(" %d" % v for v in t[0::2])
            out.append(line)
        return out


def filter_overlaps(ovl_handle, perm1, perm2, jc_bits, ic_bits, do_filter=True):
    L = load_library()
    h = c_void_p()
    p1 = np.ascontiguousarray(perm1, dtype=np.int32)
    p2 = np.ascontiguousarray(perm2, dtype=np.int32)
    L.fgb_filter.argtypes = [c_void_p, c_void_p, c_void_p, c_int, c_int, c_int, C.POINTER(c_void_p)]
    _check(L.fgb_filter(ovl_handle, _ptr(p1), _ptr(p2), jc_bits, ic_bits, int(do_filter), C.byref(h)),
           "fgb_filter")
    return _alns_out(h)


def overlaps_from_buffer(buf):
    L = load_library()
    h = c_void_p()
    buf = np.ascontiguousarray(buf, dtype=np.uint8)
    L.fgb_overlaps_from_buffer.argtypes = [c_void_p, c_ll, C.POINTER(c_void_p)]
    _check(L.fgb_overlaps_from_buffer(_ptr(buf), buf.size, C.byref(h)), "fgb_overlaps_from_buffer")
    return DeviceOverlaps(h)


class RunStats(C.Structure):
    _fields_ = [(n, c_ll) for n in ("nkmers1", "nkmers2", "nseeds", "sumlen", "nhits", "nla", "nwaves",
                                    "ncells", "nraw", "h2d_bytes", "d2h_bytes", "nseg", "nwork", "warp_cycles",
                                    "wave_cycles", "extract_cycles", "us_gix", "us_seeds", "us_extend", "us_filter",
                                    "nkmers1_fwd", "slow_cycles", "slow_waves", "paired_waves", "pairings")]

    def asdict(self):
        return {n: getattr(self, n) for n, _ in self._fields_}


DEFAULTS = dict(freq=10, chain_break=2000, chain_min=170, align_min=100, align_rate=0.3)


def _alns_out(h):
    L = load_library()
    for f in ("fgb_alns_count", "fgb_alns_raw_count", "fgb_alns_pool_bytes"):
        getattr(L, f).restype = c_ll
        getattr(L, f).argtypes = [c_void_p]
    n, nraw, pb = L.fgb_alns_count(h), L.fgb_alns_raw_count(h), L.fgb_alns_pool_bytes(h)
    fields = np.zeros((n, 9), dtype=np.int32)
    toff = np.zeros(n, dtype=np.int64)
    pool = np.zeros(max(pb, 1), dtype=np.uint8)
    L.fgb_alns_get.argtypes = [c_void_p, c_void_p, c_void_p, c_void_p]
    _check(L.fgb_alns_get(h, _ptr(fields), _ptr(toff), _ptr(pool)), "fgb_alns_get")
    L.fgb_alns_free.argtypes = [c_void_p]
    L.fgb_alns_free(h)
    return Alignments(fields, toff, pool, nraw)


def _whole_path(name, argtypes, args, stream, kw):
    p = dict(DEFAULTS)
    p.update(kw)
    L = load_library()
    h = c_void_p()
    st = RunStats()
    fn = getattr(L, name)
    fn.argtypes = argtypes + [c_int, c_int, c_int, c_int, C.c_double, C.POINTER(c_void_p), C.POINTER(RunStats),
                              c_void_p]
    _check(fn(*args, p["freq"], p["chain_break"], p["chain_min"], p["align_min"], float(p["align_rate"]),
              C.byref(h), C.byref(st), stream), name)
    return _alns_out(h), st.asdict()


def align_resident(dA, dB, freqA, stream=None, **kw):
    f = np.ascontiguousarray(freqA, dtype=np.float32)
    return _whole_path("fgb_align_resident", [c_void_p, c_void_p, c_void_p], (dA.h, dB.h, _ptr(f)), stream, kw)


def fastga_self(g, stream=None, **kw):
    f = np.ascontiguousarray(g.freq, dtype=np.float32)
    return _whole_path("fgb_fastga_self", [c_void_p, c_ll, c_int, c_void_p, c_void_p, c_void_p],
                       (_ptr(g.bps), g.bps.size, g.ncontig, _ptr(g.clen), _ptr(g.boff), _ptr(f)), stream, kw)


def fastga(gA, gB, stream=None, **kw):
    f = np.ascontiguousarray(gA.freq, dtype=np.float32)
    return _whole_path("fgb_fastga", [c_void_p, c_ll, c_int, c_void_p, c_void_p, c_void_p,
                                      c_void_p, c_ll, c_int, c_void_p, c_void_p],
                       (_ptr(gA.bps), gA.bps.size, gA.ncontig, _ptr(gA.clen), _ptr(gA.boff), _ptr(f),
                        _ptr(gB.bps), gB.bps.size, gB.ncontig, _ptr(gB.clen), _ptr(gB.boff)), stream, kw)


def compute_trace_pts(dA, dB, alns, tspace=100, stream=None, with_bad=False):
    L = load_library()
    h = c_void_p()
    fields = np.ascontiguousarray(alns.fields, dtype=np.int32)
    toff = np.ascontiguousarray(alns.toff, dtype=np.int64)
    pool = np.ascontiguousarray(alns.pool, dtype=np.uint8)
    L.fgb_compute_trace_pts.argtypes = [c_void_p, c_void_p, c_ll, c_void_p, c_void_p, c_void_p, c_int,
                                        C.POINTER(c_void_p), c_void_p]
    _check(L.fgb_compute_trace_pts(dA.h, dB.h, len(alns), _ptr(fields), _ptr(toff), _ptr(pool), tspace,
                                   C.byref(h), stream), "fgb_compute_trace_pts")
    L.fgb_scripts_total.restype = c_ll
    L.fgb_scripts_total.argtypes = [c_void_p]
    n, tot = len(alns), L.fgb_scripts_total(h)
    soff = np.zeros(n + 1, dtype=np.int64)
    script = np.zeros(max(tot, 1), dtype=np.int32)
    diffs = np.zeros(max(n, 1), dtype=np.int32)
    L.fgb_scripts_get.argtypes = [c_void_p, c_void_p, c_void_p, c_void_p]
    _check(L.fgb_scripts_get(h, _ptr(soff), _ptr(script), _ptr(diffs)), "fgb_scripts_get")
    L.fgb_scripts_bad.restype = c_ll
    L.fgb_scripts_bad.argtypes = [c_void_p]
    bad = L.fgb_scripts_bad(h)
    L.fgb_scripts_free.argtypes = [c_void_p]
    L.fgb_scripts_free(h)
    return (soff, script[:tot], diffs[:n]) + ((bad,) if with_bad else ())



def hit_groups_host(hrange, tinfo, hits, bands=1, slack=1000, gap=-1):
    L = load_library()
    hr = np.ascontiguousarray(hrange, dtype=np.uint32).reshape(-1, 2)
    ti = np.ascontiguousarray(tinfo, dtype=np.int32).reshape(-1, 2)
    hh = np.ascontiguousarray(hits, dtype=np.int64).reshape(-1, 2)
    cap = len(hh) + len(hr) + 1
    items = np.zeros((cap, 4), dtype=np.uint32)
    nxt = np.zeros((cap, 2), dtype=np.int64)
    L.fgb_hit_groups_host.restype = c_ll
    L.fgb_hit_groups_host.argtypes = [c_int, c_void_p, c_void_p, c_void_p, c_ll, c_int, c_ll, c_ll, c_void_p, c_void_p]
    n = L.fgb_hit_groups_host(len(hr), _ptr(hr), _ptr(ti), _ptr(hh), len(hh), bands, slack, gap, _ptr(items), _ptr(nxt))
    return items[:n].copy(), nxt[:n].copy()


CHAIN_TRIPLE_DT = np.dtype([("start", "i8"), ("end", "i8"), ("long", "i8"), ("key", "i8"), ("band", "i8"),
                            ("h0", "i8"), ("hn", "i8")])
CHAIN_HIT_DT = np.dtype([("alow", "i8"), ("ahgh", "i8"), ("dgmin", "i8"), ("dgmax", "i8")])
CHAIN_LISTLESS = 0x80000000


def chain_hits(seeds, chain_break=2000, chain_min=170, chunk=None, stream=None):
    L = load_library()
    L.fgb_chain_hits.argtypes = [c_void_p, c_int, c_int, c_ll, c_void_p, c_ll, c_void_p, c_ll, c_void_p, c_void_p]
    chunk = 1536 if chunk is None else int(chunk)
    info = np.zeros(6, dtype=np.int64)
    trip = np.zeros(1, dtype=CHAIN_TRIPLE_DT)
    hits = np.zeros(1, dtype=CHAIN_HIT_DT)
    for _ in range(2):
        rc = L.fgb_chain_hits(seeds.h, chain_break, chain_min, chunk, _ptr(trip), len(trip), _ptr(hits), len(hits),
                              _ptr(info), stream)
        if rc != -4:
            break
        trip = np.zeros(max(int(info[0]), 1), dtype=CHAIN_TRIPLE_DT)
        hits = np.zeros(max(int(info[2]), 1), dtype=CHAIN_HIT_DT)
    _check(rc, "fgb_chain_hits")
    names = ("work", "long", "slots", "reserved", "capacity", "chunks")
    return trip[:int(info[0])].copy(), hits[:int(info[2])].copy(), dict(zip(names, (int(v) for v in info)))


def device_free(ptr):
    L = load_library()
    L.fgb_device_free.argtypes = [c_void_p]
    L.fgb_device_free(c_void_p(ptr))


def kmers_scan(dgenome, mask, fwd_only, stream=None):
    L = load_library()
    ptr, n = c_void_p(), c_ll()
    m = np.ascontiguousarray(mask, dtype=np.uint8)
    L.fgb_kmers_scan.argtypes = [c_void_p, c_void_p, c_int, C.POINTER(c_void_p), C.POINTER(c_ll), c_void_p]
    _check(L.fgb_kmers_scan(dgenome.h, _ptr(m), int(fwd_only), C.byref(ptr), C.byref(n), stream), "fgb_kmers_scan")
    return ptr.value, n.value


def records_group_by_owner(src_ptr, n, owner256, world, dst_ptr, stream=None):
    L = load_library()
    bounds = np.zeros(world + 1, dtype=np.int64)
    own = np.ascontiguousarray(owner256, dtype=np.int32)
    assert own.shape == (256,)
    L.fgb_records_group_by_owner.argtypes = [c_void_p, c_ll, c_void_p, c_int, c_void_p, c_void_p, c_void_p]
    _check(L.fgb_records_group_by_owner(c_void_p(src_ptr), n, _ptr(own), world, c_void_p(dst_ptr), _ptr(bounds),
                                        stream), "fgb_records_group_by_owner")
    return bounds


def gix_from_records(ptr, n, plo, phi, fwd_only, post_bytes, cont_bytes, ncontig, stream=None):
    L = load_library()
    h = c_void_p()
    L.fgb_gix_from_records.argtypes = [c_void_p, c_ll, C.c_uint, C.c_uint, c_int, c_int, c_int, c_int,
                                       C.POINTER(c_void_p), c_void_p]
    _check(L.fgb_gix_from_records(c_void_p(ptr), n, plo, phi, int(fwd_only), post_bytes, cont_bytes, ncontig,
                                  C.byref(h), stream), "fgb_gix_from_records")
    return DeviceGix(h)


def seeds_merge(gix1, gix2, amxpos, bmxpos, freq=10, stream=None):
    L = load_library()
    ptr, n = c_void_p(), c_ll()
    bits = (c_int * 4)()
    info = (c_ll * 2)()
    L.fgb_seeds_merge.argtypes = [c_void_p, c_void_p, c_ll, c_ll, c_int, C.POINTER(c_void_p), C.POINTER(c_ll),
                                  c_void_p, c_void_p, c_void_p]
    _check(L.fgb_seeds_merge(gix1.h, gix2.h, amxpos, bmxpos, freq, C.byref(ptr), C.byref(n), bits, info, stream),
           "fgb_seeds_merge")
    return ptr.value, n.value, tuple(bits), info[0], info[1]


def seeds_group_by_owner(src_ptr, n, bits, owner_by_rank, world, dst_ptr, stream=None):
    L = load_library()
    bounds = np.zeros(world + 1, dtype=np.int64)
    b = (c_int * 4)(*bits)
    ow = np.ascontiguousarray(owner_by_rank, dtype=np.int32)
    L.fgb_seeds_group_by_owner.argtypes = [c_void_p, c_ll, c_void_p, c_void_p, c_int, c_int, c_void_p, c_void_p, c_void_p]
    _check(L.fgb_seeds_group_by_owner(c_void_p(src_ptr), n, b, _ptr(ow), len(ow), world, c_void_p(dst_ptr),
                                      _ptr(bounds), stream), "fgb_seeds_group_by_owner")
    return bounds


def seeds_from_records(ptr, n, bits, amxpos, bmxpos, sumlen=0, stream=None):
    L = load_library()
    h = c_void_p()
    b = (c_int * 4)(*bits)
    L.fgb_seeds_from_records.argtypes = [c_void_p, c_ll, c_void_p, c_ll, c_ll, c_ll, C.POINTER(c_void_p), c_void_p]
    _check(L.fgb_seeds_from_records(c_void_p(ptr), n, b, amxpos, bmxpos, sumlen, C.byref(h), stream),
           "fgb_seeds_from_records")
    return DeviceSeeds(h)


def local_alignments(dA, dB, jobs, freq, align_rate=0.3, tspace=100, stream=None):
    L = load_library()
    jobs = np.ascontiguousarray(jobs, dtype=np.int32).reshape(-1, 8)
    n = jobs.shape[0]
    tables, ave = align_spec(1.0 - align_rate, freq)
    paths = np.zeros((max(n, 1), 7), dtype=np.int32)
    toff = np.zeros(max(n, 1), dtype=np.int64)
    cap = 1 << 20
    L.fgb_local_alignments.argtypes = [c_void_p, c_void_p, c_ll, c_void_p, c_void_p, c_int, c_int,
                                       c_void_p, c_void_p, c_void_p, c_ll, C.POINTER(c_ll), c_void_p]
    while True:
        traces = np.zeros(cap, dtype=np.uint8)
        used = c_ll()
        rc = L.fgb_local_alignments(dA.h, dB.h, n, _ptr(jobs), _ptr(tables), ave, tspace, _ptr(paths), _ptr(toff),
                                    _ptr(traces), cap, C.byref(used), stream)
        if rc == -4 and used.value > cap:
            cap = used.value + 1024
            continue
        _check(rc, "fgb_local_alignments")
        return paths[:n], toff[:n], traces[:used.value]
```

### include/fastga_b200.h

```cpp
#ifndef FASTGA_B200_H
#define FASTGA_B200_H

#include <stdint.h>

#ifdef __cplusplus
extern "C" {
#endif

#define FGB_OK            0
#define FGB_ERR_CUDA     -1
#define FGB_ERR_ARG      -2
#define FGB_ERR_LIMIT    -3
#define FGB_ERR_OVERFLOW -4

typedef struct fgb_genome   fgb_genome;
typedef struct fgb_gix      fgb_gix;
typedef struct fgb_seeds    fgb_seeds;
typedef struct fgb_overlaps fgb_overlaps;
typedef struct fgb_alns     fgb_alns;
typedef struct fgb_scripts  fgb_scripts;

typedef struct
{ long long nkmers1, nkmers2, nseeds, sumlen, nhits, nla, nwaves, ncells, nraw, h2d_bytes, d2h_bytes,
            nseg, nwork, warp_cycles, wave_cycles, extract_cycles,
            us_gix, us_seeds, us_extend, us_filter,
            nkmers1_fwd,
            slow_cycles, slow_waves,
            paired_waves, pairings;
} fgb_run_stats;

typedef struct
{ float h2d_ms, stage_ms, scan_ms, ksort_ms, index_ms, merge_ms, ssort_ms, triples_ms, extend_ms,
        d2h_ms, filter_ms;
  int   merge_launches, extend_launches, launches;
} fgb_timings;

int fgb_fastga(const unsigned char *bpsA, long long bps_bytesA, int ncontigA, const long long *clenA,
               const long long *boffA, const float *freqA,
               const unsigned char *bpsB, long long bps_bytesB, int ncontigB, const long long *clenB,
               const long long *boffB,
               int freq, int chain_break, int chain_min, int align_min, double align_rate,
               fgb_alns **out, fgb_run_stats *stats, void *stream);

int fgb_fastga_self(const unsigned char *bps, long long bps_bytes, int ncontig, const long long *clen,
                    const long long *boff, const float *freq4,
                    int freq, int chain_break, int chain_min, int align_min, double align_rate,
                    fgb_alns **out, fgb_run_stats *stats, void *stream);

int fgb_align_resident(const fgb_genome *A, const fgb_genome *B, const float *freqA,
                       int freq, int chain_break, int chain_min, int align_min, double align_rate,
                       fgb_alns **out, fgb_run_stats *stats, void *stream);

int  fgb_genome_create(const unsigned char *bps, long long bps_bytes, int ncontig,
                       const long long *clen, const long long *boff, int want_revcomp,
                       fgb_genome **out, void *stream);
void fgb_genome_free(fgb_genome *g);
int  fgb_genome_perm(const fgb_genome *g, int *perm_out);
int  fgb_genome_download(const fgb_genome *g, int rev, unsigned long long *words, long long *woff_out);
long long fgb_genome_words(const fgb_genome *g);

int  fgb_gix_build(const fgb_genome *g, fgb_gix **out, void *stream);
int  fgb_gix_build_forward(const fgb_genome *g, fgb_gix **out, void *stream);
int  fgb_gix_build_range(const fgb_genome *g, unsigned plo, unsigned phi, fgb_gix **out, void *stream);
int  fgb_gix_upload(const void *tab, long long n, int post_bytes, int cont_bytes, int ncontig,
                    fgb_gix **out, void *stream);
int  fgb_gix_import_ktab(const unsigned char *entries, long long n, int post_bytes, int cont_bytes,
                         const long long *index, int ncontig, fgb_gix **out, void *stream);
int  fgb_gix_export_ktab(const fgb_gix *x, const long long *part_first, int nparts,
                         unsigned char *out, void *stream);
int  fgb_gix_download(const fgb_gix *x, void *tab, unsigned *pstart, unsigned long long *buck1024);
long long fgb_gix_size(const fgb_gix *x);
int  fgb_gix_post_bytes(const fgb_gix *x);
int  fgb_gix_cont_bytes(const fgb_gix *x);
void fgb_gix_free(fgb_gix *x);

int  fgb_seeds_find(const fgb_gix *x1, const fgb_gix *x2, long long amxpos, long long bmxpos,
                    int freq, fgb_seeds **out, void *stream);
int  fgb_seeds_find_self(const fgb_gix *x, long long amxpos, int freq, fgb_seeds **out, void *stream);
long long fgb_seeds_size(const fgb_seeds *s);
long long fgb_seeds_sumlen(const fgb_seeds *s);
int  fgb_seeds_layout(const fgb_seeds *s, int *bits );
int  fgb_seeds_download(const fgb_seeds *s, void *rec);
void fgb_seeds_free(fgb_seeds *s);

int  fgb_align_spec(double ave_corr, const float *freq, short *tables , int *ave_path);
int  fgb_extend(const fgb_seeds *S, const fgb_genome *A, const fgb_genome *B,
                int chain_break, int chain_min, int align_min, double align_rate,
                const short *tables, int ave_path, int tspace, fgb_overlaps **out, void *stream);
int  fgb_local_alignments(const fgb_genome *A, const fgb_genome *B, long long n, const int *jobs,
                          const short *tables, int ave_path, int tspace,
                          int *paths, long long *toff, unsigned char *traces, long long traces_cap,
                          long long *traces_used, void *stream);
int  fgb_overlaps_from_buffer(const unsigned char *buf, long long nbytes, fgb_overlaps **out);
long long fgb_overlaps_bytes(const fgb_overlaps *o);
long long fgb_overlaps_count(const fgb_overlaps *o);
const unsigned char *fgb_overlaps_data(const fgb_overlaps *o);
void fgb_overlaps_counters(const fgb_overlaps *o, unsigned long long *out );
void fgb_overlaps_retry_info(const fgb_overlaps *o, long long out[4]);
void fgb_overlaps_free(fgb_overlaps *o);

int  fgb_filter(const fgb_overlaps *O, const int *perm1, const int *perm2, int jc_bits, int ic_bits,
                int do_filter, fgb_alns **out);
long long fgb_alns_count(const fgb_alns *a);
long long fgb_alns_raw_count(const fgb_alns *a);
long long fgb_alns_pool_bytes(const fgb_alns *a);
int  fgb_alns_get(const fgb_alns *a, int *fields, long long *toff, unsigned char *pool);
void fgb_alns_free(fgb_alns *a);

int  fgb_compute_trace_pts(const fgb_genome *A, const fgb_genome *B, long long n, const int *fields,
                           const long long *toff, const unsigned char *pool, int tspace,
                           fgb_scripts **out, void *stream);
long long fgb_scripts_count(const fgb_scripts *s);
long long fgb_scripts_total(const fgb_scripts *s);
long long fgb_scripts_bad(const fgb_scripts *s);
int  fgb_scripts_get(const fgb_scripts *s, long long *soff , int *script, int *diffs );
void fgb_scripts_free(fgb_scripts *s);

int  fgb_sort128_host(void *recs, long long n, int byte_lo, int byte_hi, void *stream);
int  fgb_sort128_device(void *d_a, void *d_b, long long n, int byte_lo, int byte_hi,
                        void *d_tmp, long long tmp_bytes, int *result_in_b, void *stream);
long long fgb_sort128_tmp_bytes(long long n);

typedef struct { int beg; int end; long long off; } fgb_range;
void fgb_msd_sort(unsigned char *array, long long nelem, int rsize, int ksize,
                  long long *part, int beg, int end, int nthreads);
int  fgb_rmsd_sort(unsigned char *array, long long nelem, int rsize, int ksize, int nparts,
                   long long *part, int nthreads, fgb_range *range);

int  fgb_device_alloc(long long bytes, void **out, void *stream);
void fgb_device_free(void *p);
int  fgb_kmers_scan(const fgb_genome *g, const unsigned char *mask, int fwd_only,
                    void **d_recs, long long *n, void *stream);
int  fgb_records_group_by_owner(const void *d_recs, long long n, const int *owner256, int world,
                                void *d_out, long long *bounds, void *stream);
int  fgb_gix_from_records(const void *d_recs, long long n, unsigned plo, unsigned phi, int fwd_only,
                          int post_bytes, int cont_bytes, int ncontig, fgb_gix **out, void *stream);
int  fgb_seeds_merge(const fgb_gix *x1, const fgb_gix *x2, long long amxpos, long long bmxpos, int freq,
                     void **d_seeds, long long *n, int *bits, long long *info, void *stream);
int  fgb_seeds_group_by_owner(const void *d_seeds, long long n, const int *bits, const int *owner,
                              int nrank_contigs, int world, void *d_out, long long *bounds, void *stream);
int  fgb_seeds_from_records(const void *d_recs, long long n, const int *bits, long long amxpos,
                            long long bmxpos, long long sumlen, fgb_seeds **out, void *stream);

long long fgb_hit_groups_host(int nwork, const unsigned *hrange, const int *tinfo, const long long *hits,
                              long long nhits, int bands, long long slack, long long gap,
                              unsigned *items_out, long long *next_out);

int  fgb_chain_hits(const fgb_seeds *S, int chain_break, int chain_min, long long chunk_seeds,
                    long long *trip, long long trip_cap, long long *hits, long long hits_cap,
                    long long *info , void *stream);

int  fgb_device_ready(void);
void fgb_release_cache(void);
long long fgb_device_live_bytes(void);
void fgb_timings_reset(void);
void fgb_timings_get(fgb_timings *out);

#ifdef __cplusplus
}
#endif
#endif
```

Baseline: 4.067.

## Batch k-mer table builds for both genomes and cut host stream waits

Restructures the k-mer index build into jobs whose count, emit/sort and finish phases run for both genomes between only two stream synchronizations. Count results go into pinned host words instead of blocking copies. Per-stage event timers are now read lazily rather than synchronized on. The kmer sort now computes a device-side plan, with bin bounds found by binary search, and handles oversized buckets in a deferred pass. The aim is to remove host round-trips and idle GPU gaps during index construction, at the cost of more code complexity and memory for both jobs being live at once.

```diff
diff --git a/fastga_b200/csrc/api.cu b/fastga_b200/csrc/api.cu
--- a/fastga_b200/csrc/api.cu
+++ b/fastga_b200/csrc/api.cu
@@ -22,6 +22,40 @@
       cudaEventDestroy(a); cudaEventDestroy(b);
     }
 };
+
+struct lazy_event { cudaEvent_t a, b; float *dst; };
+static std::vector<lazy_event> g_lazy;
+static long long g_waits;
+
+struct lazy_timer
+{ lazy_event e; cudaStream_t st;
+  lazy_timer(float *d, cudaStream_t s) : st(s)
+    { e.dst = d; cudaEventCreate(&e.a); cudaEventCreate(&e.b); cudaEventRecord(e.a,st); }
+  ~lazy_timer() { cudaEventRecord(e.b,st); g_lazy.push_back(e); }
+};
+
+static void lazy_flush(bool wait)
+{ size_t k = 0;
+  for (const lazy_event &e : g_lazy)
+    { if (wait) cudaEventSynchronize(e.b);
+      else if (cudaEventQuery(e.b) != cudaSuccess) { g_lazy[k++] = e; continue; }
+      float ms = 0;
+      cudaEventElapsedTime(&ms,e.a,e.b);
+      *e.dst += ms;
+      cudaEventDestroy(e.a); cudaEventDestroy(e.b);
+    }
+  cudaGetLastError();
+  g_lazy.resize(k);
+}
+
+cudaError_t fgb_stream_wait(cudaStream_t st)
+{ g_waits += 1;
+  cudaError_t e = cudaStreamSynchronize(st);
+  lazy_flush(false);
+  return e;
+}
+
+extern "C" long long fgb_host_waits() { return g_waits; }
 
 void fgb_timing_add(int which, float ms)
 { if (which == 0) g_timings.triples_ms += ms;
@@ -99,8 +133,8 @@
   return s;
 }
 
-extern "C" void fgb_timings_reset() { memset(&g_timings,0,sizeof(g_timings)); }
-extern "C" void fgb_timings_get(fgb_timings *out) { *out = g_timings; }
+extern "C" void fgb_timings_reset() { lazy_flush(true); memset(&g_timings,0,sizeof(g_timings)); }
+extern "C" void fgb_timings_get(fgb_timings *out) { lazy_flush(true); *out = g_timings; }
 
 
 static const long long *g_sort_len;
@@ -201,102 +235,157 @@
   dblock<unsigned long long> hist;
 };
 
-static int gix_scan(const fgb_genome *g, const unsigned char *mask, unsigned plo, unsigned phi_flags,
-                    dblock<rec128> &d_recs, long long *n_out, long long *nrev, unsigned long long *buck1024,
-                    scan_layout &lay, cudaStream_t st)
-{ int T = fgb_sc_tile();
+struct gix_words
+{ u64 total, buck[1024], rdropped;
+  unsigned plan[4];
+};
+
+struct gix_job
+{ const fgb_genome *g = nullptr;
+  unsigned plo = 0, phi = 0, flags = 0;
+  bool index = true;
+  std::unique_ptr<fgb_gix> x;
+  scan_layout lay;
   std::vector<int> tc, ts;
+  int ntiles = 0;
+  dblock<int> d_tc, d_ts; dblock<unsigned> d_cnt;
+  dblock<u64> d_buck, d_total; dblock<unsigned char> d_tmp;
+  dblock<rec128> d_a, d_b; dblock<unsigned char> d_stmp, d_plan;
+  long long n = 0;
+  int inb = 0;
+  gix_words *hw = nullptr;
+};
+
+static int pinned_words(gix_job &J, int k)
+{ static thread_local gix_words *w = nullptr;
+  if (w == nullptr) CUDA_TRY(cudaHostAlloc((void **) &w,2*sizeof(gix_words),cudaHostAllocDefault));
+  J.hw = w + k;
+  return FGB_OK;
+}
+
+static int gix_job_init(gix_job &J, const fgb_genome *g, unsigned plo, unsigned phi_flags, bool index, int k)
+{ J.g = g; J.plo = plo; J.phi = phi_flags & ~GIX_FWD_ONLY; J.flags = phi_flags; J.index = index;
+  J.x.reset(new fgb_gix());
+  gix_bytes(g,J.x.get());
+  J.x->ncontig = g->ncontig;
+  J.x->fwd_only = (phi_flags & GIX_FWD_ONLY) ? 1 : 0;
+  return pinned_words(J,k);
+}
+
+static int gix_count(gix_job &J, const unsigned char *mask, cudaStream_t st)
+{ const fgb_genome *g = J.g;
+  int T = fgb_sc_tile();
   long long npos = 0;
   for (int c = 0; c < g->ncontig; c++)
     if (g->clen[c] >= 12 && g->boff[c] >= 0 && (mask == NULL || mask[c]))
       { npos += g->clen[c] - 11;
         for (long long t0 = 0; t0 + 12 <= g->clen[c]; t0 += T)
-          { tc.push_back(c); ts.push_back((int) t0); }
+          { J.tc.push_back(c); J.ts.push_back((int) t0); }
       }
-  int ntiles = (int) tc.size();
-  dblock<int> d_tc, d_ts; dblock<unsigned> d_cnt;
-  dblock<u64> d_buck, d_total; dblock<unsigned char> d_tmp;
-  int rc;
-  u64 total = 0, rdropped = 0;
-  const unsigned phi = phi_flags & ~GIX_FWD_ONLY;
-  fgb_kmer_first_digit(2*npos,plo,phi > plo ? phi : plo + 1,&lay.fsh,&lay.dbits);
-  const long long ncnt = (long long) ntiles << lay.dbits;
+  J.ntiles = (int) J.tc.size();
+  scan_layout &lay = J.lay;
+  fgb_kmer_first_digit(2*npos,J.plo,J.phi > J.plo ? J.phi : J.plo + 1,&lay.fsh,&lay.dbits);
+  const long long ncnt = (long long) J.ntiles << lay.dbits;
   const long long tmpb = fgb_dev_scan_tmp_bytes(ncnt);
   CUDA_TRY(lay.hist.alloc(256,st));
-  CUDA_TRY(d_tc.alloc(ntiles+1,st));
-  CUDA_TRY(d_ts.alloc(ntiles+1,st));
-  CUDA_TRY(d_cnt.alloc(ncnt+1,st));
-  CUDA_TRY(d_buck.alloc(1025,st));
-  CUDA_TRY(d_total.alloc(1,st));
-  CUDA_TRY(d_tmp.alloc(tmpb,st));
-  CUDA_TRY(cudaMemcpyAsync(d_tc,tc.data(),sizeof(int)*ntiles,cudaMemcpyHostToDevice,st));
-  CUDA_TRY(cudaMemcpyAsync(d_ts,ts.data(),sizeof(int)*ntiles,cudaMemcpyHostToDevice,st));
-  { stage_timer t(&g_timings.scan_ms,st);
-    rc = fgb_syncmer_digit_count_device(g->d_seq,g->d_clen,g->d_woff,g->d_crank,d_tc,d_ts,ntiles,d_buck,d_cnt,
-                                        lay.fsh,lay.dbits,lay.hist,d_total,d_tmp,tmpb,plo,phi_flags,st);
-    if (rc) return rc;
-    CUDA_TRY(cudaMemcpyAsync(&total,d_total,8,cudaMemcpyDeviceToHost,st));
-    if (buck1024) CUDA_TRY(cudaMemcpyAsync(buck1024,d_buck,8*1024,cudaMemcpyDeviceToHost,st));
-    CUDA_TRY(cudaMemcpyAsync(&rdropped,d_buck + 1024,8,cudaMemcpyDeviceToHost,st));
-    CUDA_TRY(cudaStreamSynchronize(st));
-  }
-  if (total >= 0xfffffff0ull) return FGB_ERR_LIMIT;
-  dblock<rec128> d_a;
-  CUDA_TRY(d_a.alloc(total+1,st));
-  { stage_timer t(&g_timings.scan_ms,st);
-    rc = fgb_syncmer_digit_emit_device(g->d_seq,g->d_clen,g->d_woff,g->d_crank,d_tc,d_ts,ntiles,d_cnt,lay.fsh,
-                                       lay.dbits,(long long) total,d_a,plo,phi_flags,st);
-  }
-  if (rc) return rc;
-  CUDA_TRY(cudaStreamSynchronize(st));
-  d_recs = std::move(d_a); *n_out = (long long) total; *nrev = (long long) rdropped;
-  return FGB_OK;
-}
-
-static int gix_finish(fgb_gix *x, dblock<rec128> d_a, long long n, unsigned plo, unsigned phi, const scan_layout &lay,
-                      cudaStream_t st, bool index = true)
-{ dblock<rec128> d_b; dblock<unsigned char> d_stmp;
-  long long stmpb = fgb_sort128_tmp_bytes(n);
-  int rc, inb = 0;
+  CUDA_TRY(J.d_tc.alloc(J.ntiles+1,st));
+  CUDA_TRY(J.d_ts.alloc(J.ntiles+1,st));
+  CUDA_TRY(J.d_cnt.alloc(ncnt+1,st));
+  CUDA_TRY(J.d_buck.alloc(1025,st));
+  CUDA_TRY(J.d_total.alloc(1,st));
+  CUDA_TRY(J.d_tmp.alloc(tmpb,st));
+  CUDA_TRY(cudaMemcpyAsync(J.d_tc,J.tc.data(),sizeof(int)*J.ntiles,cudaMemcpyHostToDevice,st));
+  CUDA_TRY(cudaMemcpyAsync(J.d_ts,J.ts.data(),sizeof(int)*J.ntiles,cudaMemcpyHostToDevice,st));
+  lazy_timer t(&g_timings.scan_ms,st);
+  int rc = fgb_syncmer_digit_count_device(g->d_seq,g->d_clen,g->d_woff,g->d_crank,J.d_tc,J.d_ts,J.ntiles,J.d_buck,
+                                          J.d_cnt,lay.fsh,lay.dbits,lay.hist,J.d_total,J.d_tmp,tmpb,J.plo,J.flags,st);
+  if (rc) return rc;
+  CUDA_TRY(cudaMemcpyAsync(&J.hw->total,J.d_total,8,cudaMemcpyDeviceToHost,st));
+  CUDA_TRY(cudaMemcpyAsync(J.hw->buck,J.d_buck,8*1025,cudaMemcpyDeviceToHost,st));
+  return FGB_OK;
+}
+
+static int gix_emit(gix_job &J, cudaStream_t st)
+{ if (J.hw->total >= 0xfffffff0ull) return FGB_ERR_LIMIT;
+  J.n = (long long) J.hw->total;
+  CUDA_TRY(J.d_a.alloc(J.n+1,st));
+  lazy_timer t(&g_timings.scan_ms,st);
+  return fgb_syncmer_digit_emit_device(J.g->d_seq,J.g->d_clen,J.g->d_woff,J.g->d_crank,J.d_tc,J.d_ts,J.ntiles,
+                                       J.d_cnt,J.lay.fsh,J.lay.dbits,J.n,J.d_a,J.plo,J.flags,st);
+}
+
+static int gix_sort(gix_job &J, const scan_layout &lay, cudaStream_t st)
+{ fgb_gix *x = J.x.get();
+  const long long n = J.n, stmpb = fgb_sort128_tmp_bytes(n), planb = fgb_kmer_plan_bytes(n,J.plo,J.phi,lay.fsh,lay.dbits);
+  int rc;
   x->n = n;
-  CUDA_TRY(d_b.alloc(n+1,st));
-  CUDA_TRY(d_stmp.alloc(stmpb,st));
-  if (index)
+  CUDA_TRY(J.d_b.alloc(n+1,st));
+  CUDA_TRY(J.d_stmp.alloc(stmpb,st));
+  CUDA_TRY(J.d_plan.alloc(planb,st));
+  if (J.index)
     { CUDA_TRY(x->d_pstart.alloc((1<<24)+1+8,st));
       CUDA_TRY(x->d_adj.alloc((size_t) n + 32,st));
     }
-  { stage_timer t(&g_timings.ksort_ms,st);
-    rc = fgb_kmer_sort_device(d_a,d_b,n,plo,phi,lay.fsh,lay.dbits,lay.hist,d_stmp,stmpb,&inb,st);
+  { lazy_timer t(&g_timings.ksort_ms,st);
+    rc = fgb_kmer_sort_device(J.d_a,J.d_b,n,J.plo,J.phi,lay.fsh,lay.dbits,lay.hist,J.d_stmp,stmpb,J.d_plan,&J.inb,st);
   }
   if (rc) return rc;
-  x->d_tab = std::move(inb ? d_b : d_a);
-  if (index)
-    { stage_timer t(&g_timings.index_ms,st);
-      rc = fgb_kix_index_device(x->d_tab,n,x->d_pstart,x->d_adj,st);
-    }
-  if (rc) return rc;
-  CUDA_TRY(cudaStreamSynchronize(st));
+  CUDA_TRY(cudaMemcpyAsync(J.hw->plan,J.d_plan,16,cudaMemcpyDeviceToHost,st));
+  if (J.index)
+    { lazy_timer t(&g_timings.index_ms,st);
+      rc = fgb_kix_index_device(J.inb ? J.d_b : J.d_a,n,x->d_pstart,x->d_adj,st);
+    }
+  return rc;
+}
+
+static int gix_done(gix_job &J, cudaStream_t st, fgb_gix **out)
+{ fgb_gix *x = J.x.get();
+  dblock<rec128> &tab = J.inb ? J.d_b : J.d_a;
+  int rc;
+  if (J.hw->plan[1] > 0)
+    { { lazy_timer t(&g_timings.ksort_ms,st);
+        rc = fgb_kmer_sort_oversized(J.inb ? J.d_a : J.d_b,tab,J.n,J.d_plan,J.hw->plan[1],J.hw->plan[2],st);
+      }
+      if (rc) return rc;
+      if (J.index)
+        { lazy_timer t(&g_timings.index_ms,st);
+          if ((rc = fgb_kix_index_device(tab,J.n,x->d_pstart,x->d_adj,st))) return rc;
+        }
+    }
+  x->d_tab = std::move(tab);
+  memcpy(x->buck1024,J.hw->buck,8*1024);
+  x->n_both = J.n + (long long) J.hw->rdropped;
+  *out = J.x.release();
+  return FGB_OK;
+}
+
+static const scan_layout &sort_layout(const gix_job &J)
+{ static const scan_layout none;
+  const char *part_env = getenv("FGB_KSORT_PARTITION");
+  return (part_env != NULL && atoi(part_env) != 0) ? none : J.lay;
+}
+
+static int gix_build_jobs(gix_job *J, int njob, fgb_gix **out, cudaStream_t st)
+{ int rc;
+  for (int k = 0; k < njob; k++)
+    if ((rc = gix_count(J[k],NULL,st))) return rc;
+  CUDA_TRY(fgb_stream_wait(st));
+  for (int k = 0; k < njob; k++)
+    if ((rc = gix_emit(J[k],st)) || (rc = gix_sort(J[k],sort_layout(J[k]),st))) return rc;
+  CUDA_TRY(fgb_stream_wait(st));
+  for (int k = 0; k < njob; k++)
+    if ((rc = gix_done(J[k],st,out + k))) return rc;
   return FGB_OK;
 }
 
 static int gix_build_range(const fgb_genome *g, unsigned plo, unsigned phi_flags, bool index, fgb_gix **out,
                            void *stream)
 { cudaStream_t st = (cudaStream_t) stream;
-  const unsigned phi = phi_flags & ~GIX_FWD_ONLY;
-  std::unique_ptr<fgb_gix> x(new fgb_gix());
-  gix_bytes(g,x.get());
-  x->ncontig = g->ncontig;
-  x->fwd_only = (phi_flags & GIX_FWD_ONLY) ? 1 : 0;
-  dblock<rec128> d_a; long long n = 0, nrev = 0;
-  scan_layout lay;
-  int rc = gix_scan(g,NULL,plo,phi_flags,d_a,&n,&nrev,x->buck1024,lay,st);
-  if (rc) return rc;
-  x->n_both = n + nrev;
-  const char *part_env = getenv("FGB_KSORT_PARTITION");
-  const bool ignore_layout = part_env != NULL && atoi(part_env) != 0;
-  const scan_layout none;
-  if ((rc = gix_finish(x.get(),std::move(d_a),n,plo,phi,ignore_layout ? none : lay,st,index))) return rc;
-  *out = x.release();
+  gix_job J;
+  int rc = gix_job_init(J,g,plo,phi_flags,index,0);
+  if (!rc) rc = gix_build_jobs(&J,1,out,st);
+  if (rc) return rc;
+  if (J.hw->plan[1] != 0) CUDA_TRY(fgb_stream_wait(st));
   return FGB_OK;
 }
 
@@ -314,11 +403,16 @@
 
 extern "C" int fgb_kmers_scan(const fgb_genome *g, const unsigned char *mask, int fwd_only,
                               void **d_recs, long long *n, void *stream)
-{ dblock<rec128> d; long long nrev = 0;
-  scan_layout lay;
-  int rc = gix_scan(g,mask,0u,(1u << 24) | (fwd_only ? GIX_FWD_ONLY : 0u),d,n,&nrev,NULL,lay,(cudaStream_t) stream);
-  if (rc) return rc;
-  *d_recs = d.release();
+{ cudaStream_t st = (cudaStream_t) stream;
+  gix_job J;
+  int rc = gix_job_init(J,g,0u,(1u << 24) | (fwd_only ? GIX_FWD_ONLY : 0u),false,0);
+  if (!rc) rc = gix_count(J,mask,st);
+  if (rc) return rc;
+  CUDA_TRY(fgb_stream_wait(st));
+  if ((rc = gix_emit(J,st))) return rc;
+  CUDA_TRY(fgb_stream_wait(st));
+  *n = J.n;
+  *d_recs = J.d_a.release();
   return FGB_OK;
 }
 
@@ -326,15 +420,22 @@
                                     int post_bytes, int cont_bytes, int ncontig, fgb_gix **out, void *stream)
 { cudaStream_t st = (cudaStream_t) stream;
   if (n < 0 || n >= 0xfffffff0ll || plo >= phi || phi > (1u << 24)) return FGB_ERR_ARG;
-  std::unique_ptr<fgb_gix> x(new fgb_gix());
-  x->n_both = n; x->post_bytes = post_bytes; x->cont_bytes = cont_bytes; x->ncontig = ncontig;
-  x->fwd_only = fwd_only ? 1 : 0;
-  dblock<rec128> d_a;
-  CUDA_TRY(d_a.alloc(n+1,st));
-  if (n > 0) CUDA_TRY(cudaMemcpyAsync(d_a,d_recs,sizeof(rec128)*n,cudaMemcpyDeviceToDevice,st));
-  int rc = gix_finish(x.get(),std::move(d_a),n,plo,phi,scan_layout(),st);
-  if (rc) return rc;
-  *out = x.release();
+  gix_job J;
+  J.plo = plo; J.phi = phi;
+  J.x.reset(new fgb_gix());
+  J.x->post_bytes = post_bytes; J.x->cont_bytes = cont_bytes; J.x->ncontig = ncontig;
+  J.x->fwd_only = fwd_only ? 1 : 0;
+  int rc = pinned_words(J,0);
+  if (rc) return rc;
+  J.hw->rdropped = 0;
+  memset(J.hw->buck,0,8*1024);
+  J.n = n;
+  CUDA_TRY(J.d_a.alloc(n+1,st));
+  if (n > 0) CUDA_TRY(cudaMemcpyAsync(J.d_a,d_recs,sizeof(rec128)*n,cudaMemcpyDeviceToDevice,st));
+  if ((rc = gix_sort(J,scan_layout(),st))) return rc;
+  CUDA_TRY(fgb_stream_wait(st));
+  if ((rc = gix_done(J,st,out))) return rc;
+  if (J.hw->plan[1] != 0) CUDA_TRY(fgb_stream_wait(st));
   return FGB_OK;
 }
 
@@ -603,7 +704,7 @@
 { long long nkmers1, nkmers2, nseeds, sumlen, nhits, nla, nwaves, ncells, nraw, h2d_bytes, d2h_bytes,
             nseg, nwork, warp_cycles, wave_cycles, extract_cycles,
             us_gix, us_seeds, us_extend, us_filter, nkmers1_fwd,
-            slow_cycles, slow_waves, paired_waves, pairings; };
+            slow_cycles, slow_waves, paired_waves, pairings, gix_waits; };
 
 static int align_pipeline(const fgb_genome *A, const fgb_genome *B, bool self, const float *freqA, int freq,
                           int chain_break, int chain_min, int align_min, double align_rate, fgb_alns **out,
@@ -613,13 +714,16 @@
   int rc;
   long long t0 = now_us(), t1, t2, t3, t4;
   { std::unique_ptr<fgb_gix> x1, x2;
-    fgb_gix *p = NULL;
-    if ((rc = gix_build_range(A,0u,(1u << 24) | (self ? 0u : GIX_FWD_ONLY),self,&p,st))) return rc;
-    x1.reset(p);
-    if (!self)
-      { if ((rc = gix_build_range(B,0u,1u << 24,true,&p,st))) return rc;
-        x2.reset(p);
-      }
+    fgb_gix *p[2] = { NULL, NULL };
+    const long long w0 = g_waits;
+    { gix_job J[2];
+      rc = gix_job_init(J[0],A,0u,(1u << 24) | (self ? 0u : GIX_FWD_ONLY),self,0);
+      if (!rc && !self) rc = gix_job_init(J[1],B,0u,1u << 24,true,1);
+      if (!rc) rc = gix_build_jobs(J,self ? 1 : 2,p,st);
+      x1.reset(p[0]); x2.reset(p[1]);
+      if (rc) return rc;
+    }
+    s.gix_waits = g_waits - w0;
     const fgb_gix *xb = self ? x1.get() : x2.get();
     t1 = now_us();
     s.nkmers1 = x1->n_both; s.nkmers2 = xb->n;
diff --git a/fastga_b200/csrc/common.cuh b/fastga_b200/csrc/common.cuh
--- a/fastga_b200/csrc/common.cuh
+++ b/fastga_b200/csrc/common.cuh
@@ -55,6 +55,7 @@
 
 void fgb_timing_add(int which, float ms);
 void fgb_count_launch(int n);
+cudaError_t fgb_stream_wait(cudaStream_t st);
 
 cudaError_t fgb_dmalloc(void **p, size_t bytes, cudaStream_t st);
 void fgb_dfree(void *p, cudaStream_t st);
diff --git a/fastga_b200/csrc/sort128.cu b/fastga_b200/csrc/sort128.cu
--- a/fastga_b200/csrc/sort128.cu
+++ b/fastga_b200/csrc/sort128.cu
@@ -2,6 +2,8 @@
 #include <stdlib.h>
 #include <utility>
 #include <vector>
+#include <algorithm>
+#include <stdint.h>
 
 #define SORT_THREADS 512
 #ifndef SORT_ITEMS
@@ -363,21 +365,75 @@
 #define BK_NSUB    (BK_SPAN << BK_SUBBITS)
 #define BK_MAXSUB  32
 
-__global__ void kmer_bins_kernel(const rec128 *__restrict__ tab, long long n, int binshift, unsigned long long base,
-                                 unsigned *__restrict__ bin_start, long long nbins)
-{ long long i = (long long) blockIdx.x * blockDim.x + threadIdx.x;
-  if (i > n) return;
-  long long lo = (i == 0) ? -1 : (long long) ((tab[i-1].hi >> binshift) - base);
-  long long hi = (i == n) ? nbins : (long long) ((tab[i].hi >> binshift) - base);
-  if (hi > nbins) hi = nbins;
-  for (long long p = lo+1; p <= hi; p++) bin_start[p] = (unsigned) i;
+__global__ void kmer_fine_bounds_kernel(const rec128 *__restrict__ tab, long long n, int binshift, unsigned long long base,
+                                        unsigned *__restrict__ fstart, long long nf)
+{ long long p = (long long) blockIdx.x * blockDim.x + threadIdx.x;
+  if (p > nf) return;
+  long long lo = 0, hi = n;
+  while (lo < hi)
+    { long long md = (lo + hi) >> 1;
+      if ((tab[md].hi >> binshift) - base < (unsigned long long) p) lo = md + 1; else hi = md;
+    }
+  fstart[p] = (unsigned) lo;
+}
+
+#define KP_NGROUPS 0
+#define KP_NOVER   1
+#define KP_OTOTAL  2
+struct kmer_plan
+{ unsigned *ctr, *fstart;
+  uint2 *over;
+  uint4 *groups;
+  kmer_plan(void *d, long long n, long long nf)
+    { long long ocap = n / BK_CAP + 1;
+      ctr = (unsigned *) d;
+      over = (uint2 *) (ctr + 4);
+      fstart = (unsigned *) (over + ocap);
+      groups = (uint4 *) (((uintptr_t) (fstart + nf + 1) + 15) & ~(uintptr_t) 15);
+    }
+};
+
+__global__ void kmer_plan_kernel(long long nf, long long nbins, int dsh, unsigned long long base,
+                                 unsigned long long fbase, kmer_plan P)
+{ long long p0 = ((long long) blockIdx.x * blockDim.x + threadIdx.x) * BK_SPAN;
+  if (p0 >= nbins) return;
+  const int nb = nbins - p0 < BK_SPAN ? (int) (nbins - p0) : BK_SPAN;
+  unsigned b[BK_SPAN+1];
+#pragma unroll
+  for (int k = 0; k <= BK_SPAN; k++)
+    if (k <= nb)
+      { long long f = (long long) ((base + p0 + k) << dsh) - (long long) fbase;
+        b[k] = P.fstart[f < 0 ? 0 : (f > nf ? nf : f)];
+      }
+  uint4 g[BK_SPAN];
+  int ng = 0;
+  unsigned gs = 0, gc = 0, gp = 0;
+#pragma unroll
+  for (int k = 0; k < BK_SPAN; k++)
+    { if (k >= nb) break;
+      unsigned len = b[k+1] - b[k];
+      if (len == 0) continue;
+      if (len > BK_CAP)
+        { if (gc) { g[ng++] = make_uint4(gs,gc,(unsigned) (base + p0) + gp,0); gc = 0; }
+          P.over[atomicAdd(&P.ctr[KP_NOVER],1u)] = make_uint2(b[k],len);
+          atomicAdd(&P.ctr[KP_OTOTAL],len);
+          continue;
+        }
+      if (gc + len > BK_CAP) { g[ng++] = make_uint4(gs,gc,(unsigned) (base + p0) + gp,0); gc = 0; }
+      if (gc == 0) { gs = b[k]; gp = k; }
+      gc += len;
+    }
+  if (gc) g[ng++] = make_uint4(gs,gc,(unsigned) (base + p0) + gp,0);
+  if (ng == 0) return;
+  unsigned o = atomicAdd(&P.ctr[KP_NGROUPS],(unsigned) ng);
+  for (int k = 0; k < ng; k++) P.groups[o+k] = g[k];
 }
 
 
 __global__ void __launch_bounds__(BK_THREADS,2)
 kmer_bucket_sort_kernel(const rec128 *__restrict__ in, rec128 *__restrict__ out,
                         const uint4 *__restrict__ groups ,
-                        int binshift)
+                        const unsigned *__restrict__ ngroups, int binshift)
 { extern __shared__ __align__(16) unsigned char smem_raw[];
   rec128   *tile   = reinterpret_cast<rec128 *>(smem_raw);
   unsigned *cnt    = reinterpret_cast<unsigned *>(tile + BK_CAP);
@@ -386,107 +442,116 @@
   __shared__ __align__(8) unsigned long long tbar;
 
   const int tid = threadIdx.x, lane = tid & 31, w = tid >> 5;
-  const uint4 g = groups[blockIdx.x];
-  const int count = (int) g.y;
-  if (tid == 0)
-    { mbar_init(&tbar,1);
-      tma_load_1d(tile,in + g.x,(unsigned) count * 16u,&tbar);
-    }
-  for (int i = tid; i <= BK_NSUB; i += BK_THREADS) cnt[i] = 0;
-  __syncthreads();
-  mbar_wait(&tbar,0);
-
-  rec128   r[BK_ITEMS];
-  unsigned sub[BK_ITEMS], off[BK_ITEMS];
-  const int base = w*(32*BK_ITEMS);
-  const unsigned b0 = g.z;
-  const int subshift = binshift - BK_SUBBITS;
-#pragma unroll
-  for (int it = 0; it < BK_ITEMS; it++)
-    { int idx = base + it*32 + lane;
-      if (idx < count)
-        { r[it] = ld_rec(tile + idx);
-          sub[it] = ((((unsigned) (r[it].hi >> binshift)) - b0) << BK_SUBBITS) | ((unsigned) (r[it].hi >> subshift) & ((1u << BK_SUBBITS)-1));
-          off[it] = atomicAdd(&cnt[sub[it]],1u);
-        }
-    }
-  __syncthreads();
-  bool big = false;
-  { unsigned v[8], sum = 0;
-#pragma unroll
-    for (int i = 0; i < 8; i++) { v[i] = cnt[8*tid+i]; big |= (v[i] > BK_MAXSUB); sum += v[i]; }
-    unsigned inc = warp_incl_scan(sum,lane);
-    if (lane == 31) wtot[w] = inc;
+  const unsigned ng = *ngroups;
+  if (blockIdx.x >= ng) return;
+  if (tid == 0) mbar_init(&tbar,1);
+  unsigned phase = 0;
+  for (unsigned gi = blockIdx.x; gi < ng; gi += gridDim.x, phase ^= 1)
+    {
+    const uint4 g = groups[gi];
+    const int count = (int) g.y;
+    if (tid == 0)
+      { asm volatile("fence.proxy.async.shared::cta;" ::: "memory");
+        tma_load_1d(tile,in + g.x,(unsigned) count * 16u,&tbar);
+      }
+    for (int i = tid; i <= BK_NSUB; i += BK_THREADS) cnt[i] = 0;
     __syncthreads();
-    unsigned pre = inc - sum;
-    for (int i = 0; i < w; i++) pre += wtot[i];
-#pragma unroll
-    for (int i = 0; i < 8; i++) { cnt[8*tid+i] = pre; pre += v[i]; }
-    if (tid == BK_THREADS-1) cnt[BK_NSUB] = pre;
-  }
-  big = __syncthreads_or(big);
-
-  if (!big)
-    {
-#pragma unroll
-      for (int it = 0; it < BK_ITEMS; it++)
-        { int idx = base + it*32 + lane;
-          if (idx < count) st_rec(tile + (cnt[sub[it]] + off[it]),r[it]);
-        }
+    mbar_wait(&tbar,phase);
+
+    rec128   r[BK_ITEMS];
+    unsigned sub[BK_ITEMS], off[BK_ITEMS];
+    const int base = w*(32*BK_ITEMS);
+    const unsigned b0 = g.z;
+    const int subshift = binshift - BK_SUBBITS;
+#pragma unroll
+    for (int it = 0; it < BK_ITEMS; it++)
+      { int idx = base + it*32 + lane;
+        if (idx < count)
+          { r[it] = ld_rec(tile + idx);
+            sub[it] = ((((unsigned) (r[it].hi >> binshift)) - b0) << BK_SUBBITS) | ((unsigned) (r[it].hi >> subshift) & ((1u << BK_SUBBITS)-1));
+            off[it] = atomicAdd(&cnt[sub[it]],1u);
+          }
+      }
+    __syncthreads();
+    bool big = false;
+    { unsigned v[8], sum = 0;
+#pragma unroll
+      for (int i = 0; i < 8; i++) { v[i] = cnt[8*tid+i]; big |= (v[i] > BK_MAXSUB); sum += v[i]; }
+      unsigned inc = warp_incl_scan(sum,lane);
+      if (lane == 31) wtot[w] = inc;
       __syncthreads();
-      for (int p = tid; p < count; p += BK_THREADS)
-        { rec128 R = ld_rec(tile + p);
-          unsigned sb = ((((unsigned) (R.hi >> binshift)) - b0) << BK_SUBBITS) | ((unsigned) (R.hi >> subshift) & ((1u << BK_SUBBITS)-1));
-          int s = (int) cnt[sb], e = (int) cnt[sb+1], rank = 0;
-          for (int q = s; q < e; q++)
-            { rec128 Q = ld_rec(tile + q);
-              bool less = (Q.hi < R.hi) || (Q.hi == R.hi && (Q.lo < R.lo || (Q.lo == R.lo && q < p)));
-              rank += less;
-            }
-          st_rec(out + (g.x + s + rank),R);
-        }
-      return;
-    }
-
-  unsigned *wcount = cnt;
-  unsigned *myc = wcount + w*256;
-  unsigned rank[BK_ITEMS];
-  __syncthreads();
-#pragma unroll
-  for (int i = 0; i < 8; i++) myc[i*32 + lane] = 0;
-  __syncwarp();
-  for (int byte = 0; byte < 16; byte++)
-    {
-#pragma unroll
-      for (int it = 0; it < BK_ITEMS; it++)
-        { int idx = base + it*32 + lane;
-          bool valid = idx < count;
-          rank[it] = warp_rank(myc,valid ? rec_byte(r[it],byte) : 0,valid);
-        }
-      digit_offsets(wcount,bexcl,wtot,[](unsigned) {});
-#pragma unroll
-      for (int it = 0; it < BK_ITEMS; it++)
-        { int idx = base + it*32 + lane;
-          if (idx < count)
-            { unsigned d = rec_byte(r[it],byte);
-              st_rec(tile + (bexcl[d] + myc[d] + rank[it]),r[it]);
-            }
-        }
-      __syncthreads();
-      if (byte + 1 < 16)
-        {
-#pragma unroll
-          for (int it = 0; it < BK_ITEMS; it++)
-            { int idx = base + it*32 + lane;
-              if (idx < count) r[it] = ld_rec(tile + idx);
-            }
-#pragma unroll
-          for (int i = 0; i < 8; i++) myc[i*32 + lane] = 0;
-          __syncwarp();
-        }
-    }
-  for (int p = tid; p < count; p += BK_THREADS)
-    st_rec(out + (g.x + p),ld_rec(tile + p));
+      unsigned pre = inc - sum;
+      for (int i = 0; i < w; i++) pre += wtot[i];
+#pragma unroll
+      for (int i = 0; i < 8; i++) { cnt[8*tid+i] = pre; pre += v[i]; }
+      if (tid == BK_THREADS-1) cnt[BK_NSUB] = pre;
+    }
+    big = __syncthreads_or(big);
+
+    if (!big)
+      {
+#pragma unroll
+        for (int it = 0; it < BK_ITEMS; it++)
+          { int idx = base + it*32 + lane;
+            if (idx < count) st_rec(tile + (cnt[sub[it]] + off[it]),r[it]);
+          }
+        __syncthreads();
+        for (int p = tid; p < count; p += BK_THREADS)
+          { rec128 R = ld_rec(tile + p);
+            unsigned sb = ((((unsigned) (R.hi >> binshift)) - b0) << BK_SUBBITS) | ((unsigned) (R.hi >> subshift) & ((1u << BK_SUBBITS)-1));
+            int s = (int) cnt[sb], e = (int) cnt[sb+1], rank = 0;
+            for (int q = s; q < e; q++)
+              { rec128 Q = ld_rec(tile + q);
+                bool less = (Q.hi < R.hi) || (Q.hi == R.hi && (Q.lo < R.lo || (Q.lo == R.lo && q < p)));
+                rank += less;
+              }
+            st_rec(out + (g.x + s + rank),R);
+          }
+        __syncthreads();
+        continue;
+      }
+
+    unsigned *wcount = cnt;
+    unsigned *myc = wcount + w*256;
+    unsigned rank[BK_ITEMS];
+    __syncthreads();
+#pragma unroll
+    for (int i = 0; i < 8; i++) myc[i*32 + lane] = 0;
+    __syncwarp();
+    for (int byte = 0; byte < 16; byte++)
+      {
+#pragma unroll
+        for (int it = 0; it < BK_ITEMS; it++)
+          { int idx = base + it*32 + lane;
+            bool valid = idx < count;
+            rank[it] = warp_rank(myc,valid ? rec_byte(r[it],byte) : 0,valid);
+          }
+        digit_offsets(wcount,bexcl,wtot,[](unsigned) {});
+#pragma unroll
+        for (int it = 0; it < BK_ITEMS; it++)
+          { int idx = base + it*32 + lane;
+            if (idx < count)
+              { unsigned d = rec_byte(r[it],byte);
+                st_rec(tile + (bexcl[d] + myc[d] + rank[it]),r[it]);
+              }
+          }
+        __syncthreads();
+        if (byte + 1 < 16)
+          {
+#pragma unroll
+            for (int it = 0; it < BK_ITEMS; it++)
+              { int idx = base + it*32 + lane;
+                if (idx < count) r[it] = ld_rec(tile + idx);
+              }
+#pragma unroll
+            for (int i = 0; i < 8; i++) myc[i*32 + lane] = 0;
+            __syncwarp();
+          }
+      }
+    for (int p = tid; p < count; p += BK_THREADS)
+      st_rec(out + (g.x + p),ld_rec(tile + p));
+    __syncthreads();
+    }
 }
 
 __global__ void kmer_copy_segments_kernel(const rec128 *__restrict__ src, rec128 *__restrict__ dst,
@@ -520,82 +585,33 @@
   *dbits = bits - 8*passes;
 }
 
-static int kmer_sort_binned(const rec128 *src, rec128 *dst, const unsigned *bins, long long nbins, int sh,
-                            unsigned plo, cudaStream_t st)
-{ const int binshift = 40 + sh;
-  const unsigned base = plo >> sh;
-  int rc = FGB_OK;
-  static bool attr_set = false;
-  if (!attr_set)
-    { CUDA_TRY(cudaFuncSetAttribute(kmer_bucket_sort_kernel,cudaFuncAttributeMaxDynamicSharedMemorySize,
-                                    (int) BUCKET_SMEM));
-      attr_set = true;
-    }
-
-  std::vector<uint4> groups;
-  std::vector<unsigned> ofrom, opre;
-  unsigned ototal = 0;
-  { unsigned gs = bins[0], gc = 0; long long gp = 0;
-    for (long long p = 0; p < nbins; p++)
-      { unsigned len = bins[p+1] - bins[p];
-        if (len == 0) continue;
-        if (len > BK_CAP)
-          { if (gc) { groups.push_back(make_uint4(gs,gc,base + (unsigned) gp,0)); gc = 0; }
-            ofrom.push_back(bins[p]); opre.push_back(ototal); ototal += len;
-            continue;
-          }
-        if (gc != 0 && (gc + len > BK_CAP || p - gp >= BK_SPAN))
-          { groups.push_back(make_uint4(gs,gc,base + (unsigned) gp,0)); gc = 0; }
-        if (gc == 0) { gs = bins[p]; gp = p; }
-        gc += len;
-      }
-    if (gc) groups.push_back(make_uint4(gs,gc,base + (unsigned) gp,0));
-  }
-
-  dblock<uint4> d_groups;
-  if (!groups.empty())
-    { CUDA_TRY(d_groups.alloc(groups.size(),st));
-      CUDA_TRY(cudaMemcpyAsync(d_groups,groups.data(),sizeof(uint4)*groups.size(),cudaMemcpyHostToDevice,st));
-      kmer_bucket_sort_kernel<<<(unsigned) groups.size(),BK_THREADS,BUCKET_SMEM,st>>>(src,dst,d_groups,binshift);
-      fgb_count_launch(1);
-      CUDA_TRY(cudaGetLastError());
-    }
-  if (ototal > 0)
-    { int nseg = (int) ofrom.size();
-      opre.push_back(ototal);
-      std::vector<unsigned> cfrom(opre.begin(),opre.end()-1);
-      dblock<rec128> d_c1, d_c2; dblock<unsigned char> d_ctmp; dblock<unsigned> d_seg;
-      long long ctb = fgb_sort128_tmp_bytes(ototal);
-      CUDA_TRY(d_c1.alloc((size_t) ototal+1,st));
-      CUDA_TRY(d_c2.alloc((size_t) ototal+1,st));
-      CUDA_TRY(d_ctmp.alloc(ctb,st));
-      CUDA_TRY(d_seg.alloc(3*(size_t) nseg+1,st));
-      CUDA_TRY(cudaMemcpyAsync(d_seg,ofrom.data(),sizeof(unsigned)*nseg,cudaMemcpyHostToDevice,st));
-      CUDA_TRY(cudaMemcpyAsync(d_seg+nseg,cfrom.data(),sizeof(unsigned)*nseg,cudaMemcpyHostToDevice,st));
-      CUDA_TRY(cudaMemcpyAsync(d_seg+2*nseg,opre.data(),sizeof(unsigned)*(nseg+1),cudaMemcpyHostToDevice,st));
-      int nb = (int) ((ototal + 255) / 256); if (nb > 4736) nb = 4736;
-      kmer_copy_segments_kernel<<<nb,256,0,st>>>(src,d_c1,d_seg,d_seg+nseg,d_seg+2*nseg,nseg,ototal);
-      int cinb = 0;
-      rc = fgb_sort128_device(d_c1,d_c2,ototal,0,16,d_ctmp,ctb,&cinb,st);
-      if (rc) return rc;
-      kmer_copy_segments_kernel<<<nb,256,0,st>>>(cinb ? d_c2 : d_c1,dst,d_seg+nseg,d_seg,d_seg+2*nseg,nseg,ototal);
-      fgb_count_launch(2);
-      CUDA_TRY(cudaGetLastError());
-      CUDA_TRY(cudaStreamSynchronize(st));
-    }
-  CUDA_TRY(cudaStreamSynchronize(st));
-  return FGB_OK;
+static void kmer_bins_of(long long n, unsigned plo, unsigned phi, int *fsh, int dbits, int *sh, long long *nf,
+                         long long *nbins)
+{ *sh = fgb_kmer_bin_shift(n,plo,phi);
+  if (dbits == 0) *fsh = *sh;
+  *nf = (long long) (((unsigned long long) (phi - 1) >> *fsh) - ((unsigned long long) plo >> *fsh)) + 1;
+  *nbins = (long long) (((unsigned long long) (phi - 1) >> *sh) - ((unsigned long long) plo >> *sh)) + 1;
+}
+
+extern "C" long long fgb_kmer_plan_bytes(long long n, unsigned plo, unsigned phi, int fsh, int dbits)
+{ int sh;
+  long long nf = 1, nbins = 1;
+  if (phi > plo) kmer_bins_of(n,plo,phi,&fsh,dbits,&sh,&nf,&nbins);
+  return 16 + 8*(n / BK_CAP + 1) + 4*(nf + 1) + 16 + 16*nbins;
 }
 
 extern "C" int fgb_kmer_sort_device(void *d_a, void *d_b, long long n, unsigned plo, unsigned phi, int fsh, int dbits,
-                                    const u64 *d_hist, void *d_tmp, long long tmp_bytes, int *result_in_b, void *stream)
+                                    const u64 *d_hist, void *d_tmp, long long tmp_bytes, void *d_plan,
+                                    int *result_in_b, void *stream)
 { cudaStream_t st = (cudaStream_t) stream;
   *result_in_b = 0;
+  CUDA_TRY(cudaMemsetAsync(d_plan,0,16,st));
   if (n <= 1) return FGB_OK;
   if (n >= 0xffffffffll) return FGB_ERR_LIMIT;
   if (phi <= plo || phi > (1u << 24) || tmp_bytes < fgb_sort128_tmp_bytes(n)) return FGB_ERR_ARG;
-  const int sh = fgb_kmer_bin_shift(n,plo,phi);
-  if (dbits == 0) fsh = sh;
+  int sh;
+  long long nf, nbins;
+  kmer_bins_of(n,plo,phi,&fsh,dbits,&sh,&nf,&nbins);
   if (sh < fsh) return FGB_ERR_ARG;
   const sort_tmp T(d_tmp,n);
   const int b0 = 64 + 40 + fsh + dbits, npass = (128 - b0 + 7) / 8;
@@ -612,26 +628,62 @@
       if (rc) return rc;
       std::swap(src,dst);
     }
+
+  static int grid = 0;
+  if (grid == 0)
+    { int dev, nsm, per;
+      CUDA_TRY(cudaFuncSetAttribute(kmer_bucket_sort_kernel,cudaFuncAttributeMaxDynamicSharedMemorySize,(int) BUCKET_SMEM));
+      CUDA_TRY(cudaGetDevice(&dev));
+      CUDA_TRY(cudaDeviceGetAttribute(&nsm,cudaDevAttrMultiProcessorCount,dev));
+      CUDA_TRY(cudaOccupancyMaxActiveBlocksPerMultiprocessor(&per,kmer_bucket_sort_kernel,BK_THREADS,BUCKET_SMEM));
+      grid = nsm * (per > 0 ? per : 1);
+    }
+  const kmer_plan P(d_plan,n,nf);
+  const unsigned long long base = (unsigned long long) plo >> sh, fbase = (unsigned long long) plo >> fsh;
+  const long long nwin = (nbins + BK_SPAN - 1) / BK_SPAN;
+  kmer_fine_bounds_kernel<<<(int) ((nf + 1 + 255) / 256),256,0,st>>>(src,n,40 + fsh,fbase,P.fstart,nf);
+  kmer_plan_kernel<<<(int) ((nwin + 255) / 256),256,0,st>>>(nf,nbins,sh - fsh,base,fbase,P);
+  kmer_bucket_sort_kernel<<<(unsigned) (nbins < grid ? nbins : grid),BK_THREADS,BUCKET_SMEM,st>>>(src,dst,P.groups,
+                                                                                                  P.ctr + KP_NGROUPS,
+                                                                                                  40 + sh);
+  fgb_count_launch(3);
   CUDA_TRY(cudaGetLastError());
-
-  const unsigned long long base = (unsigned long long) plo >> sh, fbase = (unsigned long long) plo >> fsh;
-  const long long nf = (long long) (((unsigned long long) (phi - 1) >> fsh) - fbase) + 1;
-  const long long nbins = (long long) (((unsigned long long) (phi - 1) >> sh) - base) + 1;
-  std::vector<unsigned> fstart((size_t) nf + 1), bins((size_t) nbins + 1);
-  { dblock<unsigned> d_fstart;
-    CUDA_TRY(d_fstart.alloc((size_t) (nf+1),st));
-    kmer_bins_kernel<<<(int) ((n + 1 + 255) / 256),256,0,st>>>(src,n,40 + fsh,fbase,d_fstart,nf);
-    fgb_count_launch(1);
-    CUDA_TRY(cudaMemcpyAsync(fstart.data(),d_fstart,sizeof(unsigned)*(size_t) (nf+1),cudaMemcpyDeviceToHost,st));
-    CUDA_TRY(cudaStreamSynchronize(st));
-  }
-  for (long long p = 0; p <= nbins; p++)
-    { long long f = (long long) ((base + p) << (sh - fsh)) - (long long) fbase;
-      bins[p] = fstart[f < 0 ? 0 : (f > nf ? nf : f)];
-    }
-  int rc = kmer_sort_binned(src,dst,bins.data(),nbins,sh,plo,st);
+  *result_in_b = (dst == (rec128 *) d_b);
+  return FGB_OK;
+}
+
+extern "C" int fgb_kmer_sort_oversized(const void *src, void *dst, long long n, const void *d_plan, unsigned nover,
+                                       unsigned ototal, void *stream)
+{ cudaStream_t st = (cudaStream_t) stream;
+  if (nover == 0) return FGB_OK;
+  const kmer_plan P(const_cast<void *>(d_plan),n,0);
+  std::vector<uint2> over(nover);
+  CUDA_TRY(cudaMemcpyAsync(over.data(),P.over,sizeof(uint2)*nover,cudaMemcpyDeviceToHost,st));
+  CUDA_TRY(fgb_stream_wait(st));
+  std::sort(over.begin(),over.end(),[](const uint2 &x, const uint2 &y) { return x.x < y.x; });
+  const int nseg = (int) nover;
+  std::vector<unsigned> ofrom(nseg), opre(nseg + 1);
+  opre[0] = 0;
+  for (int k = 0; k < nseg; k++) { ofrom[k] = over[k].x; opre[k+1] = opre[k] + over[k].y; }
+  if (opre[nseg] != ototal) return FGB_ERR_ARG;
+  dblock<rec128> d_c1, d_c2; dblock<unsigned char> d_ctmp; dblock<unsigned> d_seg;
+  long long ctb = fgb_sort128_tmp_bytes(ototal);
+  CUDA_TRY(d_c1.alloc((size_t) ototal+1,st));
+  CUDA_TRY(d_c2.alloc((size_t) ototal+1,st));
+  CUDA_TRY(d_ctmp.alloc(ctb,st));
+  CUDA_TRY(d_seg.alloc(3*(size_t) nseg+1,st));
+  CUDA_TRY(cudaMemcpyAsync(d_seg,ofrom.data(),sizeof(unsigned)*nseg,cudaMemcpyHostToDevice,st));
+  CUDA_TRY(cudaMemcpyAsync(d_seg+nseg,opre.data(),sizeof(unsigned)*nseg,cudaMemcpyHostToDevice,st));
+  CUDA_TRY(cudaMemcpyAsync(d_seg+2*nseg,opre.data(),sizeof(unsigned)*(nseg+1),cudaMemcpyHostToDevice,st));
+  int nb = (int) ((ototal + 255) / 256); if (nb > 4736) nb = 4736;
+  kmer_copy_segments_kernel<<<nb,256,0,st>>>((const rec128 *) src,d_c1,d_seg,d_seg+nseg,d_seg+2*nseg,nseg,ototal);
+  int cinb = 0;
+  int rc = fgb_sort128_device(d_c1,d_c2,ototal,0,16,d_ctmp,ctb,&cinb,st);
   if (rc) return rc;
-  *result_in_b = (dst == (rec128 *) d_b);
+  kmer_copy_segments_kernel<<<nb,256,0,st>>>(cinb ? d_c2 : d_c1,(rec128 *) dst,d_seg+nseg,d_seg,d_seg+2*nseg,nseg,ototal);
+  fgb_count_launch(2);
+  CUDA_TRY(cudaGetLastError());
+  CUDA_TRY(fgb_stream_wait(st));
   return FGB_OK;
 }
 
diff --git a/fastga_b200/csrc/stages.h b/fastga_b200/csrc/stages.h
--- a/fastga_b200/csrc/stages.h
+++ b/fastga_b200/csrc/stages.h
@@ -16,9 +16,12 @@
                        void *d_tmp, long long tmp_bytes, int *result_in_b, void *stream);
 int fgb_kmer_bin_shift(long long n, unsigned plo, unsigned phi);
 void fgb_kmer_first_digit(long long nmax, unsigned plo, unsigned phi, int *fsh, int *dbits);
+long long fgb_kmer_plan_bytes(long long n, unsigned plo, unsigned phi, int fsh, int dbits);
 int fgb_kmer_sort_device(void *d_a, void *d_b, long long n, unsigned plo, unsigned phi, int fsh, int dbits,
-                         const unsigned long long *d_hist, void *d_tmp, long long tmp_bytes, int *result_in_b,
-                         void *stream);
+                         const unsigned long long *d_hist, void *d_tmp, long long tmp_bytes, void *d_plan,
+                         int *result_in_b, void *stream);
+int fgb_kmer_sort_oversized(const void *src, void *dst, long long n, const void *d_plan, unsigned nover,
+                            unsigned ototal, void *stream);
 
 int fgb_stage_genome_device(const void *d_bps, const long long *d_boff, const long long *d_clen,
                             const long long *d_woff, int ncontig, long long total_words,
diff --git a/fastga_b200/lib.py b/fastga_b200/lib.py
--- a/fastga_b200/lib.py
+++ b/fastga_b200/lib.py
@@ -35,6 +35,12 @@
 
 def timings_reset():
     load_library().fgb_timings_reset()
+
+
+def host_waits():
+    L = load_library()
+    L.fgb_host_waits.restype = c_ll
+    return L.fgb_host_waits()
 
 
 def timings_get():
@@ -416,7 +422,8 @@
     _fields_ = [(n, c_ll) for n in ("nkmers1", "nkmers2", "nseeds", "sumlen", "nhits", "nla", "nwaves",
                                     "ncells", "nraw", "h2d_bytes", "d2h_bytes", "nseg", "nwork", "warp_cycles",
                                     "wave_cycles", "extract_cycles", "us_gix", "us_seeds", "us_extend", "us_filter",
-                                    "nkmers1_fwd", "slow_cycles", "slow_waves", "paired_waves", "pairings")]
+                                    "nkmers1_fwd", "slow_cycles", "slow_waves", "paired_waves", "pairings",
+                                    "gix_waits")]
 
     def asdict(self):
         return {n: getattr(self, n) for n, _ in self._fields_}
diff --git a/include/fastga_b200.h b/include/fastga_b200.h
--- a/include/fastga_b200.h
+++ b/include/fastga_b200.h
@@ -26,7 +26,8 @@
             us_gix, us_seeds, us_extend, us_filter,
             nkmers1_fwd,
             slow_cycles, slow_waves,
-            paired_waves, pairings;
+            paired_waves, pairings,
+            gix_waits;
 } fgb_run_stats;
 
 typedef struct
@@ -155,6 +156,7 @@
 long long fgb_device_live_bytes(void);
 void fgb_timings_reset(void);
 void fgb_timings_get(fgb_timings *out);
+long long fgb_host_waits(void);
 
 #ifdef __cplusplus
 }
diff --git a/profiles/kmer_wait_bench.py b/profiles/kmer_wait_bench.py
--- /dev/null
+++ b/profiles/kmer_wait_bench.py
@@ -0,0 +1,96 @@
+#!/usr/bin/env python
+import argparse
+import filecmp
+import json
+import os
+import subprocess
+import sys
+import tempfile
+
+import numpy as np
+
+ROOT = os.path.dirname(os.path.dirname(os.path.abspath(__file__)))
+
+
+def gpu_info():
+    try:
+        out = subprocess.run(["nvidia-smi", "--query-gpu=name,power.limit,clocks.max.sm", "--format=csv,noheader"],
+                             stdout=subprocess.PIPE, text=True, check=True).stdout.strip().split("\n")[0]
+        name, power, mhz = [s.strip() for s in out.split(",")]
+        return {"name": name, "power_limit": power, "sm_max_clock": mhz}
+    except Exception as ex:
+        return {"error": str(ex)[:200]}
+
+
+def run_bench(lib, steps, warmup, reference, dump):
+    env = dict(os.environ, FGB_LIB=os.path.abspath(lib))
+    cmd = [sys.executable, os.path.join(ROOT, "bench.py"), "--gpus", "1", "--steps", str(steps),
+           "--warmup", str(warmup)]
+    if not reference:
+        cmd.append("--no-cpu-baseline")
+    if dump:
+        cmd += ["--dump-outputs", dump]
+    out = subprocess.run(cmd, env=env, stdout=subprocess.PIPE, text=True, check=True, cwd=ROOT).stdout
+    line = json.loads([s for s in out.splitlines() if s.startswith("{")][-1])
+    c = line["config"]
+    st, hw = c["stage_ms"], c["host_wall_us"]
+    return {"step_ms": c["step_ms_min_med_max"][1], "step_ms_min_med_max": c["step_ms_min_med_max"],
+            "us_gix": hw["us_gix"] / 1000.0, "scan_ms": st["scan_ms"], "ksort_ms": st["ksort_ms"],
+            "index_ms": st["index_ms"], "kmers": c["kmers"], "seeds": c["seeds"], "hits": c["hits"], "triples": c["triples"],
+            "waves": c["waves"], "aln_md5": c["aln_md5"], "gpu_launches": line["gpu_launches"],
+            "parity_equal": line.get("parity", {}).get("equal")}
+
+
+def dumps_identical(da, db):
+    fa, fb = sorted(os.listdir(da)), sorted(os.listdir(db))
+    return fa == fb and len(fa) > 0 and all(filecmp.cmp(os.path.join(da, f), os.path.join(db, f), shallow=False)
+                                            for f in fa)
+
+
+def main():
+    ap = argparse.ArgumentParser()
+    ap.add_argument("--lib-a", required=True, help="the parent build")
+    ap.add_argument("--lib-b", required=True, help="this build")
+    ap.add_argument("--pairs", type=int, default=6)
+    ap.add_argument("--steps", type=int, default=10)
+    ap.add_argument("--warmup", type=int, default=3)
+    ap.add_argument("--out", default=None, help="also write the runs here (JSON)")
+    args = ap.parse_args()
+
+    runs = []
+    with tempfile.TemporaryDirectory() as tmp:
+        for p in range(args.pairs):
+            pair = {}
+            for tag, lib in (("a", args.lib_a), ("b", args.lib_b)):
+                dump = os.path.join(tmp, tag) if p == 0 else None
+                pair[tag] = run_bench(lib, args.steps, args.warmup, p == 0, dump)
+            if p == 0:
+                pair["dumps_identical"] = dumps_identical(os.path.join(tmp, "a"), os.path.join(tmp, "b"))
+            runs.append(pair)
+            print(json.dumps({"pair": p, **pair}), file=sys.stderr)
+
+    def col(tag, k):
+        return np.array([r[tag][k] for r in runs], dtype=float)
+
+    same = all(r["a"][k] == r["b"][k] for r in runs for k in ("kmers", "seeds", "hits", "triples", "waves", "aln_md5"))
+    summary = {}
+    for k in ("us_gix", "scan_ms", "ksort_ms", "index_ms", "step_ms"):
+        a, b = col("a", k), col("b", k)
+        summary[k] = {"a_median": float(np.median(a)), "b_median": float(np.median(b)),
+                      "a_min_max": [float(a.min()), float(a.max())], "b_min_max": [float(b.min()), float(b.max())],
+                      "b_lower_in_every_pair": bool((b < a).all()), "pair_diff_min_max": [float((a - b).min()),
+                                                                                          float((a - b).max())]}
+    line = {"what": "k-mer table builds of the bench pair (bench.py --gpus 1), build a vs b alternating",
+            "gpu": gpu_info(), "lib_a": os.path.basename(args.lib_a), "lib_b": os.path.basename(args.lib_b),
+            "pairs": args.pairs, "steps": args.steps, "warmup": args.warmup,
+            "outputs_same": same, "dumps_identical": runs[0].get("dumps_identical"),
+            "parity_equal": [runs[0]["a"]["parity_equal"], runs[0]["b"]["parity_equal"]],
+            "summary": summary}
+    if args.out:
+        with open(args.out, "w") as f:
+            json.dump({"summary": line, "runs": runs}, f, indent=1)
+    print(json.dumps(line))
+
+
+if __name__ == "__main__":
+    main()
```

Measured after the change: 4.307, median of 6. +5.9%, better.
